# ESandML/SSL4GIE

Measured on AMD Instinct MI355X. Metric: images/sec/GPU (fwd+bwd) ViT-B 224² bs=256 at 1/2/4/8 MI355X; % MFMA peak, higher is better.
Workload: dtype bf16; 1 GPU; ViT-B MAE pretrain (mae_vit_base_patch16, norm_pix_loss, mask 0.75) fwd+bwd+grad-allreduce+AdamW, 224x224 synthetic N(0,1) images resident in HBM; batch_per_gpu=256, global_batch=256, parallelism=dp1, optimizer=AdamW(0.9,0.95) wd 0.05 (ssl4gie_amd.optim.ArenaAdamW)

## Files before the change

include/ssl4gie_hip.h:

```cpp
#ifndef SSL4GIE_HIP_H
#define SSL4GIE_HIP_H
#include <stddef.h>
#include <stdint.h>
#ifdef __cplusplus
extern "C" {
#endif

#define SSL4GIE_F32 0
#define SSL4GIE_BF16 1
#define SSL4GIE_EARG 1000
#define SSL4GIE_EPEER 1001

int ssl4gie_abi_version(void);

int ssl4gie_layernorm_fwd(const float* x, const float* gamma, const float* beta, void* y,
                          int y_dtype, float* mean, float* rstd, int rows, int cols, float eps,
                          void* stream);
size_t ssl4gie_layernorm_bwd_workspace_bytes(int rows, int cols);
int ssl4gie_layernorm_bwd(const void* dy, int dy_dtype, const float* x, const float* gamma,
                          const float* mean, const float* rstd, const float* dres, float* dx,
                          void* dx_lp, int lp_dtype, float* dgamma, float* dbeta, int accumulate,
                          float* workspace, int rows, int cols, void* stream);

size_t ssl4gie_colsum_workspace_bytes(int rows, int cols);
int ssl4gie_colsum(const void* x, int dtype, float* out, int accumulate, float* workspace,
                   int rows, int cols, long long ld, void* stream);

enum {
    SSL4GIE_EPI_NONE = 0,
    SSL4GIE_EPI_BIAS = 1,
    SSL4GIE_EPI_BIAS_GELU = 2,
    SSL4GIE_EPI_BIAS_RESIDUAL = 3,
    SSL4GIE_EPI_DGELU = 4,
    SSL4GIE_EPI_BIAS_GELU_GRAD = 5,
    SSL4GIE_EPI_MUL_AUX = 6,
    SSL4GIE_EPI_RELU_MASK_AUX = 7,
    SSL4GIE_EPI_ADD_AUX = 8,
    SSL4GIE_EPI_AFFINE_AUX_RELU = 9
};
typedef struct ssl4gie_conv3x3_geom {
    int B, H, W, C;
    int stride;
    int relu;
} ssl4gie_conv3x3_geom;

typedef struct ssl4gie_gemm_desc {
    int M, N, K;
    int batch1, batch2;
    const void* A;
    long long sAm, sAk, sAb1, sAb2;
    const void* B;
    long long sBk, sBn, sBb1, sBb2;
    void* C;
    long long ldc, sCb1, sCb2;
    int dtype_ab;
    int dtype_c;
    float alpha;
    int epilogue;
    const float* bias;
    const float* residual;
    long long ldr;
    const void* aux;
    void* out2;
    int accumulate;
    float* colsum_a;
    const ssl4gie_conv3x3_geom* conv;
    float* colstats;
    const float* scale;
    int relu;
} ssl4gie_gemm_desc;
size_t ssl4gie_gemm_workspace_bytes(const ssl4gie_gemm_desc* d);
int ssl4gie_gemm(const ssl4gie_gemm_desc* d, void* workspace, size_t workspace_bytes,
                 void* stream);
size_t ssl4gie_gemm_tn_pair_workspace_bytes(const ssl4gie_gemm_desc* a, const ssl4gie_gemm_desc* b);
int ssl4gie_gemm_tn_pair(const ssl4gie_gemm_desc* a, const ssl4gie_gemm_desc* b, void* workspace,
                         size_t workspace_bytes, void* stream);
size_t ssl4gie_gemm_tn_group_workspace_bytes(const ssl4gie_gemm_desc* descs, int n);
int ssl4gie_gemm_tn_group(const ssl4gie_gemm_desc* descs, int n, void* workspace,
                          size_t workspace_bytes, void* stream);

size_t ssl4gie_attn_workspace_bytes(int dtype, int B, int N, int H, int hd);
int ssl4gie_attn_fwd(const void* qkv, void* out, float* lse, int dtype, int B, int N, int H,
                     int hd, void* workspace, void* stream);
int ssl4gie_attn_bwd(const void* qkv, const void* out, const void* dout, const float* lse,
                     void* dqkv, int dtype, int B, int N, int H, int hd, void* workspace,
                     void* stream);

int ssl4gie_cast(const float* src, void* dst, int dst_dtype, long long n, void* stream);
int ssl4gie_cast_transpose(const float* src, void* dst, int dst_dtype, int rows, int cols,
                           void* stream);
int ssl4gie_cast_transpose_batch(const float* src, void* dst, const long long* mat_off,
                                 const int* mat_rows, const int* mat_cols, const int* tile_start,
                                 int S, int total_tiles, void* stream);
int ssl4gie_add_cast(const float* a, const float* b, float* out, void* out_lp, int lp_dtype,
                     long long n, void* stream);

int ssl4gie_mask_argsort(const float* noise, long long* ids_shuffle, long long* ids_restore,
                         float* mask, int B, int L, int len_keep, void* stream);
int ssl4gie_patch_gather(const float* img, const long long* ids, void* out, int out_dtype,
                         int B, int C, int H, int W, int p, int nsel, long long ids_stride,
                         int order, void* stream);
int ssl4gie_tokens_assemble(const void* y, int y_dtype, const float* cls, const float* pos,
                            const long long* ids, long long ids_stride, float* x, int B,
                            int nsel, int D, void* stream);
int ssl4gie_tokens_assemble_bwd(const float* dx, void* dy, int dy_dtype, float* dcls,
                                int accumulate, int B, int nsel, int D, void* stream);
int ssl4gie_decoder_assemble(const void* y, int y_dtype, const float* mask_token,
                             const float* dpos, const long long* ids_restore, float* xd, int B,
                             int L, int nkeep, int D, void* stream);
size_t ssl4gie_decoder_assemble_bwd_workspace_bytes(int B, int L, int D);
int ssl4gie_decoder_assemble_bwd(const float* dxd, const long long* ids_shuffle, void* dy,
                                 int dy_dtype, float* dmask_token, int accumulate,
                                 float* workspace, int B, int L, int nkeep, int D, void* stream);
int ssl4gie_mae_loss(const float* pred, const float* img, const float* mask, float* per_patch,
                     float* dpred, const float* gpp, float gscale_host, int norm_pix,
                     int has_cls, int B, int C, int H, int W, int p, void* stream);

typedef struct ssl4gie_block_weights {
    const float *ln1_g, *ln1_b, *ln2_g, *ln2_b;
    const float *bqkv, *bproj, *bfc1, *bfc2;
    const void *wqkv, *wproj, *wfc1, *wfc2;
    const void *wqkv_t, *wproj_t, *wfc1_t, *wfc2_t;
} ssl4gie_block_weights;
typedef struct ssl4gie_block_grads {
    float *ln1_g, *ln1_b, *ln2_g, *ln2_b;
    float *bqkv, *bproj, *bfc1, *bfc2;
    float *wqkv, *wproj, *wfc1, *wfc2;
} ssl4gie_block_grads;
typedef struct ssl4gie_block_act {
    float *mean1, *rstd1, *mean2, *rstd2;
    void* h1;
    void* qkv;
    void* attn;
    float* lse;
    float* xmid;
    void* h2;
    void* u;
    void* g;
} ssl4gie_block_act;
typedef struct ssl4gie_block_dims {
    int B, N, D, H, F;
    int dtype;
    float eps;
} ssl4gie_block_dims;
size_t ssl4gie_block_workspace_bytes(const ssl4gie_block_dims* d);
int ssl4gie_block_fwd(const ssl4gie_block_dims* d, const ssl4gie_block_weights* w,
                      const ssl4gie_block_act* a, const float* x_in, float* x_out,
                      void* workspace, void* stream);
#define SSL4GIE_BWD_ACCUMULATE 1
#define SSL4GIE_BWD_DEFER_WGRAD 2
#define SSL4GIE_BWD_NO_JOIN 4
#define SSL4GIE_BWD_SLOT(s) (((s) & 3) << 4)
int ssl4gie_block_bwd(const ssl4gie_block_dims* d, const ssl4gie_block_weights* w,
                      const ssl4gie_block_act* a, const ssl4gie_block_grads* g,
                      const float* x_in, const float* dx_out, const void* dx_out_lp,
                      float* dx_in, void* dx_in_lp, int accumulate, void* workspace,
                      void* stream);
int ssl4gie_set_wgrad_stream(int on);
int ssl4gie_block_wgrad_descs(const ssl4gie_block_dims* d, const ssl4gie_block_act* a,
                              const ssl4gie_block_grads* g, const void* dy, void* workspace,
                              int accumulate, ssl4gie_gemm_desc* out4);
int ssl4gie_wgrad_group(const ssl4gie_gemm_desc* descs, int n, void* workspace, size_t workspace_bytes,
                        int slot, void* stream);
int ssl4gie_wgrad_wait(int slot, void* stream);
int ssl4gie_set_compute_cus(int n);

int ssl4gie_conv3x3_weight_pack(const float* w, void* out, int dtype, int Cout, int Cin, int mode, int ld,
                                void* stream);
int ssl4gie_conv3x3_weight_pack_batch(const void* const* w, void* const* out, const int* Cout, const int* Cin,
                                      const int* mode, const int* ld, int n, int dtype, void* stream);
int ssl4gie_conv3x3_wgrad_unpack(const float* dw2, float* dw, int Cout, int Cin, int ld, int accumulate,
                                 void* stream);
int ssl4gie_im2col3x3(const void* x, void* cols, int dtype, int B, int H, int W, int C, int stride,
                      int relu, long long ld, void* stream);
int ssl4gie_col2im3x3(const void* dcols, void* dx, int dtype, int B, int H, int W, int C,
                      int stride, long long ld, void* stream);
int ssl4gie_conv3x3_direct_ok(int B, int H, int W, int Cin, int Cout);
int ssl4gie_conv3x3_direct_tiles(int B, int H, int W);
int ssl4gie_conv3x3_direct_fwd(const void* x, const void* w2, const float* bias,
                               const void* relu_mask, void* y, float* colstats, int B, int H, int W,
                               int Cin, int Cout, int relu_in, void* stream);
int ssl4gie_conv3x3_direct_wgrad_ok(int B, int H, int W, int Cin, int Cout);
size_t ssl4gie_conv3x3_direct_wgrad_workspace_bytes(int B, int H, int W, int Cin, int Cout);
int ssl4gie_conv3x3_direct_wgrad(const void* dy, const void* x, float* dw2, float* dbias,
                                 void* workspace, size_t workspace_bytes, int B, int H, int W, int Cin,
                                 int Cout, int relu_in, int accumulate, void* stream);
int ssl4gie_conv3x3_direct_fwd_affine(const void* x, const float* in_coef, const void* w2, const float* bias,
                                      void* y, float* colstats, int B, int H, int W, int Cin, int Cout,
                                      int relu_in, void* stream);
int ssl4gie_conv3x3_direct_wgrad_affine(const void* dy, const void* x, const float* in_coef, float* dw2,
                                        float* dbias, void* workspace, size_t workspace_bytes, int B, int H,
                                        int W, int Cin, int Cout, int relu_in, int accumulate, void* stream);
size_t ssl4gie_stem7x7_packed_bytes(int B, int H, int W);
int ssl4gie_stem7x7_pack(const float* img, void* packed, int B, int H, int W, void* stream);
int ssl4gie_stem7x7_tiles(int B, int H, int W);
int ssl4gie_stem7x7_fwd(const void* packed, const void* w2s, void* y, float* colstats, int B, int H,
                        int W, void* stream);
size_t ssl4gie_stem7x7_wgrad_workspace_bytes(int B, int H, int W);
int ssl4gie_stem7x7_wgrad(const void* dy, const void* packed, float* dw2s, void* workspace,
                          size_t workspace_bytes, int B, int H, int W, int accumulate, void* stream);
int ssl4gie_bilinear2x_fwd(const void* x, void* y, int dtype, int B, int H, int W, int C,
                           void* stream);
int ssl4gie_bilinear2x_bwd(const void* dy, void* dx, int dtype, int B, int H, int W, int C,
                           void* stream);
int ssl4gie_pixel_shuffle(const void* g, const float* bias, void* y, int dtype, int B, int H, int W,
                          int k, int C, void* stream);
int ssl4gie_pixel_unshuffle(const void* dy, void* dg, int dtype, int B, int H, int W, int k, int C,
                            void* stream);
int ssl4gie_tokens_to_map(const float* z, void* x, int dtype, int B, int L, int D, void* stream);
int ssl4gie_map_to_tokens(const void* dx, float* dz, int dtype, int B, int L, int D, void* stream);
int ssl4gie_eltwise(int op, const void* a, const void* b, const void* c, void* out, int dtype,
                    long long n, void* stream);
int ssl4gie_depth_head_fwd(const void* x, const float* w, const float* bias, float* y, int dtype,
                           long long M, int C, void* stream);
size_t ssl4gie_depth_head_bwd_workspace_bytes(long long M, int C);
int ssl4gie_depth_head_bwd(const void* x, const float* w, const float* y, const float* dy, void* dx,
                           float* dw, float* db, int accumulate, float* workspace, int dtype,
                           long long M, int C, void* stream);

int ssl4gie_stem_im2col7x7(const float* img, void* cols, int dtype, int B, int H, int W,
                           long long ld, void* stream);
int ssl4gie_subsample2(const void* x, void* y, int dtype, int B, int H, int W, int C, int backward,
                       void* stream);
size_t ssl4gie_bn_workspace_bytes(long long rows, int C);
int ssl4gie_bn_fwd(const void* x, const float* gamma, const float* beta, const void* res, void* y,
                   float* mean, float* rstd, float* running_mean, float* running_var,
                   float momentum, float eps, int relu, int training, float* workspace, int dtype,
                   long long rows, int C, void* stream);
int ssl4gie_bn_bwd(const void* dy, const void* y, const void* x, const float* gamma,
                   const float* mean, const float* rstd, void* dx, void* dres, float* dgamma,
                   float* dbeta, int accumulate, int relu, float* workspace, int dtype,
                   long long rows, int C, void* stream);
int ssl4gie_bn_bwd_xmask(const void* dy, const void* x, const float* gamma, const float* beta,
                         const float* mean, const float* rstd, void* dx, float* dgamma, float* dbeta,
                         int accumulate, float* workspace, int dtype, long long rows, int C, void* stream);
int ssl4gie_bn_fwd_partials_bits(const void* x, const float* partial, int parts, const float* gamma,
                                 const float* beta, const void* res, void* y, unsigned char* relu_bits,
                                 float* mean, float* rstd, float* running_mean, float* running_var,
                                 float momentum, float eps, float* workspace, int dtype, long long rows, int C,
                                 void* stream);
int ssl4gie_bn_bwd_bits(const void* dy, const unsigned char* relu_bits, const void* x, const float* gamma,
                        const float* mean, const float* rstd, void* dx, void* dres, float* dgamma, float* dbeta,
                        int accumulate, float* workspace, int dtype, long long rows, int C, void* stream);
int ssl4gie_bn_stats(const void* x, float* mean, float* var, float* workspace, int dtype,
                     long long rows, int C, void* stream);
int ssl4gie_bn_combine_stats(const float* gathered, int world, int C, float eps, float momentum,
                             float* running_mean, float* running_var, float* mean, float* rstd, float* total,
                             void* stream);
int ssl4gie_bn_bwd_reduce(const void* dy, const void* y, const void* x, const float* mean,
                          const float* rstd, void* dres, float* sums, int relu, float* workspace,
                          int dtype, long long rows, int C, void* stream);
int ssl4gie_bn_bwd_apply(const void* dy, const void* y, const void* x, const float* gamma,
                         const float* mean, const float* rstd, const float* sums, float inv_count,
                         void* dx, int relu, float* workspace, int dtype, long long rows, int C,
                         void* stream);
int ssl4gie_bn_bwd_reduce_xmask(const void* dy, const void* x, const float* gamma, const float* beta,
                                const float* mean, const float* rstd, float* sums, float* workspace, int dtype,
                                long long rows, int C, void* stream);
int ssl4gie_bn_bwd_apply_xmask(const void* dy, const void* x, const float* gamma, const float* beta,
                               const float* mean, const float* rstd, const float* sums, float inv_count, void* dx,
                               float* workspace, int dtype, long long rows, int C, void* stream);
int ssl4gie_bn_coef_stats(const float* mean, const float* rstd, const float* gamma, const float* beta, float* coef,
                          int C, void* stream);
int ssl4gie_bn_apply_bits(const void* x, const float* coef, const void* res, void* y, unsigned char* relu_bits,
                          int dtype, long long rows, int C, void* stream);
int ssl4gie_bn_bwd_reduce_bits(const void* dy, const unsigned char* relu_bits, const void* x, const float* mean,
                               const float* rstd, void* dres, float* sums, float* workspace, int dtype,
                               long long rows, int C, void* stream);
int ssl4gie_ema_update(float* dst, const float* src, float m, long long n, void* stream);
int ssl4gie_bn_fwd_partials(const void* x, const float* partial, int parts, const float* gamma,
                            const float* beta, const void* res, void* y, float* mean, float* rstd,
                            float* running_mean, float* running_var, float momentum, float eps,
                            int relu, float* workspace, int dtype, long long rows, int C,
                            void* stream);
int ssl4gie_bn_coef_partials(const float* partial, int parts, const float* gamma, const float* beta,
                             float* mean, float* rstd, float* running_mean, float* running_var,
                             float momentum, float eps, float* coef, float* workspace, long long rows, int C,
                             void* stream);
int ssl4gie_bn_stats_partials(const float* partial, int parts, float* mean, float* var,
                              float* workspace, long long rows, int C, void* stream);
int ssl4gie_maxpool3x3s2_fwd(const void* x, void* y, unsigned char* arg, int dtype, int B, int H,
                             int W, int C, void* stream);
int ssl4gie_maxpool3x3s2_bwd(const void* dy, const unsigned char* arg, void* dx, int dtype, int B,
                             int H, int W, int C, void* stream);
int ssl4gie_bn_maxpool3x3s2_fwd(const void* x, const float* coef, int relu, void* y, unsigned char* arg,
                                int dtype, int B, int H, int W, int C, void* stream);
int ssl4gie_avgpool_fwd(const void* x, float* y, int dtype, int B, int HW, int C, void* stream);
int ssl4gie_avgpool_bwd(const float* dy, void* dx, int dtype, int B, int HW, int C, void* stream);

int ssl4gie_adamw_arena(float* p, const float* g, float* m, float* v, const long long* seg_start,
                        const float* seg_lr, const float* seg_wd, int S, float beta1, float beta2,
                        float eps, int step, long long n, void* stream);
int ssl4gie_adamw_arena_lp(float* p, const float* g, float* m, float* v, const long long* seg_start,
                           const float* seg_lr, const float* seg_wd, int S, float beta1, float beta2,
                           float eps, int step, long long n, void* lp_bf16, void* stream);
int ssl4gie_adamw_arena_range(float* p, const float* g, float* m, float* v, const long long* seg_start,
                              const float* seg_lr, const float* seg_wd, int S, float beta1, float beta2,
                              float eps, int step, long long lo, long long hi, void* lp_bf16,
                              void* stream);
size_t ssl4gie_lars_workspace_bytes(int S);
int ssl4gie_lars_arena(float* p, const float* g, float* mu, const long long* seg_start,
                       const float* seg_lr, const float* seg_wd, const float* seg_mat, int S,
                       float momentum, float trust, float* workspace, long long n, void* stream);

int ssl4gie_normalize_u8(const unsigned char* img, float* out, const float* mean, const float* std,
                         int B, int H, int W, void* stream);

int ssl4gie_maxpool2x2_fwd(const void* x, void* y, int dtype, int B, int H, int W, int C,
                           void* stream);
int ssl4gie_maxpool2x2_bwd(const void* x, const void* dy, void* dx, int dtype, int B, int H, int W,
                           int C, void* stream);
int ssl4gie_gelu_map(const void* x, const void* dy, void* out, int dtype, long long n, void* stream);
size_t ssl4gie_map_layernorm_workspace_bytes(int B);
int ssl4gie_map_layernorm_fwd(const void* x, const float* w, const float* bias, void* y, float* mean,
                              float* rstd, float eps, float* workspace, int dtype, int B, long long M,
                              void* stream);
int ssl4gie_map_layernorm_bwd(const void* x, const void* dy, const float* w, const float* mean,
                              const float* rstd, void* dx, float* dw, float* db, int accumulate,
                              float* workspace, int dtype, int B, long long M, void* stream);

#define SSL4GIE_PROF_KINDS 7
int ssl4gie_prof_begin(int max_launches);
int ssl4gie_prof_collect(double* ms, double* flops, long long* launches);
int ssl4gie_prof_end(void);

size_t ssl4gie_ssi_loss_workspace_bytes(int B, int H, int W);
int ssl4gie_ssi_loss(const float* pred, const float* target, float* loss, float* dpred, int B, int H,
                     int W, float alpha, int scales, void* workspace, void* stream);
size_t ssl4gie_dice_loss_workspace_bytes(int B);
int ssl4gie_dice_loss(const float* logits, const float* target, float* loss, float* dlogits, int B,
                      long long n, float smooth, void* workspace, void* stream);

int ssl4gie_debug_nt256_stamps(void* dst, size_t bytes);

typedef struct ssl4gie_ar_handle ssl4gie_ar_handle;
size_t ssl4gie_allreduce_direct_blob_bytes(void);
int ssl4gie_allreduce_direct_init(int rank, int world, size_t max_elems, void* export_blob,
                                  ssl4gie_ar_handle** out);
int ssl4gie_allreduce_direct_connect(ssl4gie_ar_handle* h, const void* all_blobs);
int ssl4gie_allreduce_direct_enqueue(ssl4gie_ar_handle* h, float* grad, size_t n_elems, float scale,
                                     void* stream);
int ssl4gie_allgather_direct_enqueue(ssl4gie_ar_handle* h, const float* src, size_t n_elems, float* dst,
                                     void* stream);
unsigned ssl4gie_allreduce_direct_error(const ssl4gie_ar_handle* h);
int ssl4gie_allreduce_direct_set_timeout(ssl4gie_ar_handle* h, double seconds);
int ssl4gie_allreduce_direct_destroy(ssl4gie_ar_handle* h);

#ifdef __cplusplus
}
#endif
#endif
```

ssl4gie_amd/_lib.py:

```python
from __future__ import annotations

import ctypes as C
import os

_HERE = os.path.dirname(os.path.abspath(__file__))
LIB_PATH = os.path.join(_HERE, "libssl4gie_hip.so")
_dbg = os.environ.get("SSL4GIE_DEBUG_LIB", "")
if _dbg == "1" or _dbg.startswith("x"):
    LIB_PATH = os.path.join(_HERE, "libssl4gie_hip_dbg.so" if _dbg == "1" else f"libssl4gie_hip_{_dbg}.so")
    import sys as _sys
    print(f"ssl4gie_amd: SSL4GIE_DEBUG_LIB=1 -> loading the DEBUG library {LIB_PATH}", file=_sys.stderr)

ABI_VERSION = 7

PROF_KINDS = 7

F32, BF16 = 0, 1
BWD_ACCUMULATE, BWD_DEFER_WGRAD, BWD_NO_JOIN = 1, 2, 4
EPI_NONE, EPI_BIAS, EPI_BIAS_GELU, EPI_BIAS_RESIDUAL, EPI_DGELU, EPI_BIAS_GELU_GRAD, EPI_MUL_AUX, \
    EPI_RELU_MASK_AUX, EPI_ADD_AUX, EPI_AFFINE_AUX_RELU = range(10)

vp, i32, i64, f32, sz = C.c_void_p, C.c_int, C.c_longlong, C.c_float, C.c_size_t


class Conv3x3Geom(C.Structure):
    _fields_ = [("B", i32), ("H", i32), ("W", i32), ("C", i32), ("stride", i32), ("relu", i32)]


class GemmDesc(C.Structure):
    _fields_ = [
        ("M", i32), ("N", i32), ("K", i32), ("batch1", i32), ("batch2", i32),
        ("A", vp), ("sAm", i64), ("sAk", i64), ("sAb1", i64), ("sAb2", i64),
        ("B", vp), ("sBk", i64), ("sBn", i64), ("sBb1", i64), ("sBb2", i64),
        ("C", vp), ("ldc", i64), ("sCb1", i64), ("sCb2", i64),
        ("dtype_ab", i32), ("dtype_c", i32), ("alpha", f32), ("epilogue", i32),
        ("bias", vp), ("residual", vp), ("ldr", i64), ("aux", vp), ("out2", vp),
        ("accumulate", i32), ("colsum_a", vp), ("conv", C.POINTER(Conv3x3Geom)),
        ("colstats", vp), ("scale", vp), ("relu", i32),
    ]


_W_F32 = ("ln1_g", "ln1_b", "ln2_g", "ln2_b", "bqkv", "bproj", "bfc1", "bfc2")
_W_LP = ("wqkv", "wproj", "wfc1", "wfc2", "wqkv_t", "wproj_t", "wfc1_t", "wfc2_t")
_G_ALL = _W_F32 + ("wqkv", "wproj", "wfc1", "wfc2")
_ACT = ("mean1", "rstd1", "mean2", "rstd2", "h1", "qkv", "attn", "lse", "xmid", "h2", "u", "g")


class BlockWeights(C.Structure):
    _fields_ = [(n, vp) for n in _W_F32 + _W_LP]


class BlockGrads(C.Structure):
    _fields_ = [(n, vp) for n in _G_ALL]


class BlockAct(C.Structure):
    _fields_ = [(n, vp) for n in _ACT]


class BlockDims(C.Structure):
    _fields_ = [("B", i32), ("N", i32), ("D", i32), ("H", i32), ("F", i32), ("dtype", i32),
                ("eps", f32)]


PROTOTYPES = {
    "ssl4gie_abi_version": (i32, []),
    "ssl4gie_layernorm_fwd": (i32, [vp, vp, vp, vp, i32, vp, vp, i32, i32, f32, vp]),
    "ssl4gie_layernorm_bwd_workspace_bytes": (sz, [i32, i32]),
    "ssl4gie_layernorm_bwd": (i32, [vp, i32, vp, vp, vp, vp, vp, vp, vp, i32, vp, vp, i32, vp,
                                    i32, i32, vp]),
    "ssl4gie_colsum_workspace_bytes": (sz, [i32, i32]),
    "ssl4gie_colsum": (i32, [vp, i32, vp, i32, vp, i32, i32, i64, vp]),
    "ssl4gie_gemm_workspace_bytes": (sz, [C.POINTER(GemmDesc)]),
    "ssl4gie_gemm": (i32, [C.POINTER(GemmDesc), vp, sz, vp]),
    "ssl4gie_attn_workspace_bytes": (sz, [i32, i32, i32, i32, i32]),
    "ssl4gie_attn_fwd": (i32, [vp, vp, vp, i32, i32, i32, i32, i32, vp, vp]),
    "ssl4gie_attn_bwd": (i32, [vp, vp, vp, vp, vp, i32, i32, i32, i32, i32, vp, vp]),
    "ssl4gie_cast": (i32, [vp, vp, i32, i64, vp]),
    "ssl4gie_cast_transpose": (i32, [vp, vp, i32, i32, i32, vp]),
    "ssl4gie_cast_transpose_batch": (i32, [vp, vp, vp, vp, vp, vp, i32, i32, vp]),
    "ssl4gie_add_cast": (i32, [vp, vp, vp, vp, i32, i64, vp]),
    "ssl4gie_mask_argsort": (i32, [vp, vp, vp, vp, i32, i32, i32, vp]),
    "ssl4gie_patch_gather": (i32, [vp, vp, vp, i32, i32, i32, i32, i32, i32, i32, i64, i32, vp]),
    "ssl4gie_tokens_assemble": (i32, [vp, i32, vp, vp, vp, i64, vp, i32, i32, i32, vp]),
    "ssl4gie_tokens_assemble_bwd": (i32, [vp, vp, i32, vp, i32, i32, i32, i32, vp]),
    "ssl4gie_decoder_assemble": (i32, [vp, i32, vp, vp, vp, vp, i32, i32, i32, i32, vp]),
    "ssl4gie_decoder_assemble_bwd_workspace_bytes": (sz, [i32, i32, i32]),
    "ssl4gie_decoder_assemble_bwd": (i32, [vp, vp, vp, i32, vp, i32, vp, i32, i32, i32, i32, vp]),
    "ssl4gie_mae_loss": (i32, [vp, vp, vp, vp, vp, vp, f32, i32, i32, i32, i32, i32, i32, i32, vp]),
    "ssl4gie_im2col3x3": (i32, [vp, vp, i32, i32, i32, i32, i32, i32, i32, i64, vp]),
    "ssl4gie_col2im3x3": (i32, [vp, vp, i32, i32, i32, i32, i32, i32, i64, vp]),
    "ssl4gie_conv3x3_direct_ok": (i32, [i32, i32, i32, i32, i32]),
    "ssl4gie_conv3x3_direct_tiles": (i32, [i32, i32, i32]),
    "ssl4gie_conv3x3_direct_fwd": (i32, [vp, vp, vp, vp, vp, vp, i32, i32, i32, i32, i32, i32, vp]),
    "ssl4gie_conv3x3_direct_wgrad_ok": (i32, [i32, i32, i32, i32, i32]),
    "ssl4gie_conv3x3_direct_wgrad_workspace_bytes": (sz, [i32, i32, i32, i32, i32]),
    "ssl4gie_conv3x3_direct_wgrad": (i32, [vp, vp, vp, vp, vp, sz, i32, i32, i32, i32, i32, i32, i32, vp]),
    "ssl4gie_conv3x3_direct_wgrad_affine": (i32, [vp, vp, vp, vp, vp, vp, sz, i32, i32, i32, i32, i32, i32, i32, vp]),
    "ssl4gie_conv3x3_direct_fwd_affine": (i32, [vp, vp, vp, vp, vp, vp, i32, i32, i32, i32, i32, i32, vp]),
    "ssl4gie_stem7x7_packed_bytes": (sz, [i32, i32, i32]),
    "ssl4gie_stem7x7_pack": (i32, [vp, vp, i32, i32, i32, vp]),
    "ssl4gie_stem7x7_tiles": (i32, [i32, i32, i32]),
    "ssl4gie_stem7x7_fwd": (i32, [vp, vp, vp, vp, i32, i32, i32, vp]),
    "ssl4gie_stem7x7_wgrad_workspace_bytes": (sz, [i32, i32, i32]),
    "ssl4gie_stem7x7_wgrad": (i32, [vp, vp, vp, vp, sz, i32, i32, i32, i32, vp]),
    "ssl4gie_bilinear2x_fwd": (i32, [vp, vp, i32, i32, i32, i32, i32, vp]),
    "ssl4gie_bilinear2x_bwd": (i32, [vp, vp, i32, i32, i32, i32, i32, vp]),
    "ssl4gie_pixel_shuffle": (i32, [vp, vp, vp, i32, i32, i32, i32, i32, i32, vp]),
    "ssl4gie_pixel_unshuffle": (i32, [vp, vp, i32, i32, i32, i32, i32, i32, vp]),
    "ssl4gie_tokens_to_map": (i32, [vp, vp, i32, i32, i32, i32, vp]),
    "ssl4gie_map_to_tokens": (i32, [vp, vp, i32, i32, i32, i32, vp]),
    "ssl4gie_eltwise": (i32, [i32, vp, vp, vp, vp, i32, i64, vp]),
    "ssl4gie_depth_head_fwd": (i32, [vp, vp, vp, vp, i32, i64, i32, vp]),
    "ssl4gie_depth_head_bwd_workspace_bytes": (sz, [i64, i32]),
    "ssl4gie_depth_head_bwd": (i32, [vp, vp, vp, vp, vp, vp, vp, i32, vp, i32, i64, i32, vp]),
    "ssl4gie_stem_im2col7x7": (i32, [vp, vp, i32, i32, i32, i32, i64, vp]),
    "ssl4gie_subsample2": (i32, [vp, vp, i32, i32, i32, i32, i32, i32, vp]),
    "ssl4gie_bn_workspace_bytes": (sz, [i64, i32]),
    "ssl4gie_bn_fwd": (i32, [vp, vp, vp, vp, vp, vp, vp, vp, vp, f32, f32, i32, i32, vp, i32, i64, i32, vp]),
    "ssl4gie_bn_bwd": (i32, [vp, vp, vp, vp, vp, vp, vp, vp, vp, vp, i32, i32, vp, i32, i64, i32, vp]),
    "ssl4gie_bn_stats": (i32, [vp, vp, vp, vp, i32, i64, i32, vp]),
    "ssl4gie_bn_fwd_partials_bits": (i32, [vp, vp, i32, vp, vp, vp, vp, vp, vp, vp, vp, vp, f32, f32, vp, i32, i64,
                                           i32, vp]),
    "ssl4gie_bn_bwd_bits": (i32, [vp, vp, vp, vp, vp, vp, vp, vp, vp, vp, i32, vp, i32, i64, i32, vp]),
    "ssl4gie_bn_bwd_xmask": (i32, [vp, vp, vp, vp, vp, vp, vp, vp, vp, i32, vp, i32, i64, i32, vp]),
    "ssl4gie_bn_bwd_reduce_xmask": (i32, [vp, vp, vp, vp, vp, vp, vp, vp, i32, i64, i32, vp]),
    "ssl4gie_bn_bwd_apply_xmask": (i32, [vp, vp, vp, vp, vp, vp, vp, f32, vp, vp, i32, i64, i32, vp]),
    "ssl4gie_bn_bwd_reduce": (i32, [vp, vp, vp, vp, vp, vp, vp, i32, vp, i32, i64, i32, vp]),
    "ssl4gie_bn_coef_stats": (i32, [vp, vp, vp, vp, vp, i32, vp]),
    "ssl4gie_bn_apply_bits": (i32, [vp, vp, vp, vp, vp, i32, i64, i32, vp]),
    "ssl4gie_bn_bwd_reduce_bits": (i32, [vp, vp, vp, vp, vp, vp, vp, vp, i32, i64, i32, vp]),
    "ssl4gie_bn_bwd_apply": (i32, [vp, vp, vp, vp, vp, vp, vp, f32, vp, i32, vp, i32, i64, i32, vp]),
    "ssl4gie_ema_update": (i32, [vp, vp, f32, i64, vp]),
    "ssl4gie_maxpool3x3s2_fwd": (i32, [vp, vp, vp, i32, i32, i32, i32, i32, vp]),
    "ssl4gie_bn_maxpool3x3s2_fwd": (i32, [vp, vp, i32, vp, vp, i32, i32, i32, i32, i32, vp]),
    "ssl4gie_maxpool3x3s2_bwd": (i32, [vp, vp, vp, i32, i32, i32, i32, i32, vp]),
    "ssl4gie_avgpool_fwd": (i32, [vp, vp, i32, i32, i32, i32, vp]),
    "ssl4gie_avgpool_bwd": (i32, [vp, vp, i32, i32, i32, i32, vp]),
    "ssl4gie_bn_coef_partials": (i32, [vp, i32, vp, vp, vp, vp, vp, vp, f32, f32, vp, vp, i64, i32, vp]),
    "ssl4gie_bn_fwd_partials": (i32, [vp, vp, i32, vp, vp, vp, vp, vp, vp, vp, vp, f32, f32, i32, vp, i32, i64,
                                      i32, vp]),
    "ssl4gie_bn_stats_partials": (i32, [vp, i32, vp, vp, vp, i64, i32, vp]),
    "ssl4gie_adamw_arena": (i32, [vp, vp, vp, vp, vp, vp, vp, i32, f32, f32, f32, i32, i64, vp]),
    "ssl4gie_adamw_arena_lp": (i32, [vp, vp, vp, vp, vp, vp, vp, i32, f32, f32, f32, i32, i64, vp, vp]),
    "ssl4gie_adamw_arena_range": (i32, [vp, vp, vp, vp, vp, vp, vp, i32, f32, f32, f32, i32, i64, i64, vp, vp]),
    "ssl4gie_lars_workspace_bytes": (sz, [i32]),
    "ssl4gie_lars_arena": (i32, [vp, vp, vp, vp, vp, vp, vp, i32, f32, f32, vp, i64, vp]),
    "ssl4gie_normalize_u8": (i32, [vp, vp, C.POINTER(C.c_float), C.POINTER(C.c_float), i32, i32, i32, vp]),
    "ssl4gie_maxpool2x2_fwd": (i32, [vp, vp, i32, i32, i32, i32, i32, vp]),
    "ssl4gie_maxpool2x2_bwd": (i32, [vp, vp, vp, i32, i32, i32, i32, i32, vp]),
    "ssl4gie_gelu_map": (i32, [vp, vp, vp, i32, i64, vp]),
    "ssl4gie_map_layernorm_workspace_bytes": (sz, [i32]),
    "ssl4gie_map_layernorm_fwd": (i32, [vp, vp, vp, vp, vp, vp, f32, vp, i32, i32, i64, vp]),
    "ssl4gie_map_layernorm_bwd": (i32, [vp, vp, vp, vp, vp, vp, vp, vp, i32, vp, i32, i32, i64, vp]),
    "ssl4gie_gemm_tn_pair_workspace_bytes": (sz, [vp, vp]),
    "ssl4gie_gemm_tn_pair": (i32, [vp, vp, vp, sz, vp]),
    "ssl4gie_gemm_tn_group_workspace_bytes": (sz, [vp, i32]),
    "ssl4gie_gemm_tn_group": (i32, [vp, i32, vp, sz, vp]),
    "ssl4gie_block_wgrad_descs": (i32, [C.POINTER(BlockDims), C.POINTER(BlockAct), C.POINTER(BlockGrads), vp, vp,
                                        i32, vp]),
    "ssl4gie_wgrad_group": (i32, [vp, i32, vp, sz, i32, vp]),
    "ssl4gie_wgrad_wait": (i32, [i32, vp]),
    "ssl4gie_set_wgrad_stream": (i32, [i32]),
    "ssl4gie_set_compute_cus": (i32, [i32]),
    "ssl4gie_ssi_loss_workspace_bytes": (sz, [i32, i32, i32]),
    "ssl4gie_ssi_loss": (i32, [vp, vp, vp, vp, i32, i32, i32, f32, i32, vp, vp]),
    "ssl4gie_dice_loss_workspace_bytes": (sz, [i32]),
    "ssl4gie_dice_loss": (i32, [vp, vp, vp, vp, i32, i64, f32, vp, vp]),
    "ssl4gie_allreduce_direct_blob_bytes": (sz, []),
    "ssl4gie_allreduce_direct_init": (i32, [i32, i32, sz, vp, C.POINTER(vp)]),
    "ssl4gie_allreduce_direct_connect": (i32, [vp, vp]),
    "ssl4gie_allreduce_direct_enqueue": (i32, [vp, vp, sz, f32, vp]),
    "ssl4gie_allgather_direct_enqueue": (i32, [vp, vp, sz, vp, vp]),
    "ssl4gie_bn_combine_stats": (i32, [vp, i32, i32, f32, f32, vp, vp, vp, vp, vp, vp]),
    "ssl4gie_allreduce_direct_error": (C.c_uint, [vp]),
    "ssl4gie_allreduce_direct_set_timeout": (i32, [vp, C.c_double]),
    "ssl4gie_allreduce_direct_destroy": (i32, [vp]),
    "ssl4gie_conv3x3_weight_pack_batch": (i32, [vp, vp, vp, vp, vp, vp, i32, i32, vp]),
    "ssl4gie_conv3x3_weight_pack": (i32, [vp, vp, i32, i32, i32, i32, i32, vp]),
    "ssl4gie_conv3x3_wgrad_unpack": (i32, [vp, vp, i32, i32, i32, i32, vp]),
    "ssl4gie_debug_nt256_stamps": (i32, [vp, sz]),
    "ssl4gie_prof_begin": (i32, [i32]),
    "ssl4gie_prof_collect": (i32, [vp, vp, vp]),
    "ssl4gie_prof_end": (i32, []),
    "ssl4gie_block_workspace_bytes": (sz, [C.POINTER(BlockDims)]),
    "ssl4gie_block_fwd": (i32, [C.POINTER(BlockDims), C.POINTER(BlockWeights),
                                C.POINTER(BlockAct), vp, vp, vp, vp]),
    "ssl4gie_block_bwd": (i32, [C.POINTER(BlockDims), C.POINTER(BlockWeights),
                                C.POINTER(BlockAct), C.POINTER(BlockGrads), vp, vp, vp, vp, vp,
                                i32, vp, vp]),
}

_lib = None


class HipExtensionMissing(RuntimeError):
    pass


def load():
    global _lib
    if _lib is not None:
        return _lib
    if not os.path.exists(LIB_PATH):
        raise HipExtensionMissing(
            f"{LIB_PATH} not found: build it with `make -C ssl4gie_amd/csrc` "
            "(or `python -c 'import __graft_entry__ as g; g.build()'`). "
            "ssl4gie_amd has no CPU / eager fallback.")
    lib = C.CDLL(LIB_PATH)
    for name, (res, args) in PROTOTYPES.items():
        fn = getattr(lib, name)
        fn.restype = res
        fn.argtypes = args
    got = lib.ssl4gie_abi_version()
    if got != ABI_VERSION:
        raise HipExtensionMissing(
            f"{LIB_PATH} has ABI revision {got}, this package binds revision {ABI_VERSION}: "
            "rebuild it (`make -C ssl4gie_amd/csrc`)")
    _lib = lib
    return lib


def check(rc: int, what: str):
    if rc != 0:
        kind = {1000: "invalid argument",
                1001: "a peer of the direct all-reduce did not arrive in time (sticky)"}.get(rc, f"hipError_t {rc}")
        raise RuntimeError(f"libssl4gie_hip: {what} failed ({kind})")
```

ssl4gie_amd/csrc/gemm256.h:

```cpp
#pragma once
#include "gemm_internal.h"

#define P_BM 256
#define P_BN 256
#define P_BK 64
#define P_HALF 16384
#define P_BUF 65536
#define P_STG_WAVE 4096
#define P_LDS_BYTES (2 * P_BUF + 8 * P_STG_WAVE)

DEVI int p_swz(int r) { return (r >> 1) & 7; }

DEVI unsigned p_lds_addr(const void* p) {
    return (unsigned)(uintptr_t)(__attribute__((address_space(3))) const char*)p;
}

DEVI void p_glds2(const void* sbase, unsigned v0, unsigned v1, unsigned l0, unsigned l1) {
    unsigned keep;
    asm volatile(
        "s_mov_b32 %0, m0\n\t"
        "s_mov_b32 m0, %4\n\t"
        "s_nop 0\n\t"
        "global_load_lds_dwordx4 %2, %1\n\t"
        "s_mov_b32 m0, %5\n\t"
        "s_nop 0\n\t"
        "global_load_lds_dwordx4 %3, %1\n\t"
        "s_mov_b32 m0, %0"
        : "=&s"(keep)
        : "s"(sbase), "v"(v0), "v"(v1), "s"(l0), "s"(l1)
        : "memory");
}

DEVI void p_glds1(const void* sbase, unsigned v0, unsigned l0) {
    unsigned keep;
    asm volatile(
        "s_mov_b32 %0, m0\n\t"
        "s_mov_b32 m0, %3\n\t"
        "s_nop 0\n\t"
        "global_load_lds_dwordx4 %2, %1\n\t"
        "s_mov_b32 m0, %0"
        : "=&s"(keep)
        : "s"(sbase), "v"(v0), "s"(l0)
        : "memory");
}

DEVI void p_glds1_dword(const void* sbase, unsigned v0, unsigned l0) {
    unsigned keep;
    asm volatile(
        "s_mov_b32 %0, m0\n\t"
        "s_mov_b32 m0, %3\n\t"
        "s_nop 0\n\t"
        "global_load_lds_dword %2, %1\n\t"
        "s_mov_b32 m0, %0"
        : "=&s"(keep)
        : "s"(sbase), "v"(v0), "s"(l0)
        : "memory");
}

DEVI void p_glds2v(const void* a0, const void* a1, unsigned l0, unsigned l1) {
    unsigned keep;
    asm volatile(
        "s_mov_b32 %0, m0\n\t"
        "s_mov_b32 m0, %3\n\t"
        "s_nop 0\n\t"
        "global_load_lds_dwordx4 %1, off\n\t"
        "s_mov_b32 m0, %4\n\t"
        "s_nop 0\n\t"
        "global_load_lds_dwordx4 %2, off\n\t"
        "s_mov_b32 m0, %0"
        : "=&s"(keep)
        : "v"(a0), "v"(a1), "s"(l0), "s"(l1)
        : "memory");
}

DEVI unsigned p_fastdiv(unsigned n, unsigned mg, unsigned sh) { return __umulhi(n, mg) >> sh; }

DEVI bf16x8 p_relu8(bf16x8 v) {
    typedef __attribute__((ext_vector_type(8))) short s16x8_t;
    const s16x8_t z = {0, 0, 0, 0, 0, 0, 0, 0};
    return __builtin_bit_cast(bf16x8, __builtin_elementwise_max(__builtin_bit_cast(s16x8_t, v), z));
}

#ifndef P_EPI_XPOSE_SWAP
#define P_EPI_XPOSE_SWAP true
#endif
#ifndef P_EPI_PRIO_MODE
#define P_EPI_PRIO_MODE 0
#endif
#define P_MFMA(a, b, c) __builtin_amdgcn_mfma_f32_16x16x32_bf16((a), (b), (c), 0, 0, 0)

template <bool NT, class V> DEVI void est(V* p, V v) {
    if constexpr (NT) __builtin_nontemporal_store(v, p);
    else *p = v;
}
template <bool NT> DEVI void est4(float* p, f32x4 v) { est<NT>((f32x4*)p, v); }
template <bool NT> DEVI void est4(bf16_t* p, f32x4 v) {
    u32x2 r;
    r[0] = pack_bf2(v[0], v[1]);
    r[1] = pack_bf2(v[2], v[3]);
    est<NT>((u32x2*)p, r);
}

template <bool FULL, bool RESID, int NJ = 4, bool NT = false>
DEVI void p_store_f32(f32x4 (&acc)[8][4], char* stg, const float alpha, const f32x4 bias_t ,
                      const float* __restrict__ residual, const long long ldr, const bool accumulate,
                      float* __restrict__ C, const long long ldc, int rbase, int cbase, int M, int N,
                      int lane) {
    const int r16 = lane & 15, g4 = lane >> 4;
    const int R0 = lane >> 4, Cc = lane & 15;
    const int gn = cbase + 4 * Cc;
    const bool mine = NJ == 4 || Cc < 4 * NJ;
    constexpr int PF = NJ == 3 ? 3 : 2;
    f32x4 rs[PF][4];
    auto fetch = [&](int mt, f32x4 (&dst)[4]) {
#pragma unroll
        for (int q = 0; q < 4; ++q) {
            const int gm = rbase + 16 * mt + R0 + 4 * q;
            dst[q] = (mine && (FULL || (gm < M && gn < N))) ? ld4(residual + (size_t)gm * ldr + gn)
                                                            : f32x4{0, 0, 0, 0};
        }
    };
    if constexpr (RESID) {
#pragma unroll
        for (int mt = 0; mt < PF; ++mt) fetch(mt, rs[mt]);
    }
    auto put = [&](int mt) {
#pragma unroll
        for (int nt = 0; nt < NJ; ++nt) {
            const f32x4 v = acc[mt][nt] * alpha;
            const int c = nt * 4 + g4;
            *(f32x4*)(stg + r16 * 256 + ((c ^ r16) << 4)) = v;
        }
    };
    put(0);
#pragma unroll
    for (int mt = 0; mt < 8; ++mt) {
        f32x4 w[4];
#pragma unroll
        for (int q = 0; q < 4; ++q) {
            const int R = R0 + 4 * q;
            w[q] = *(const f32x4*)(stg + R * 256 + ((Cc ^ R) << 4));
        }
        __builtin_amdgcn_sched_barrier(0);
        if (mt + 1 < 8) put(mt + 1);
        __builtin_amdgcn_sched_barrier(0);
#pragma unroll
        for (int q = 0; q < 4; ++q) {
            const int R = R0 + 4 * q;
            const int gm = rbase + 16 * mt + R;
            w[q] += bias_t;
            if constexpr (RESID) w[q] += rs[mt % PF][q];
            if (mine && (FULL || (gm < M && gn < N))) {
                float* c = C + (size_t)gm * ldc + gn;
                if (accumulate) w[q] += ld4(c);
                est4<NT>(c, w[q]);
            }
        }
        if constexpr (RESID) {
            if (mt + PF < 8) fetch(mt + PF, rs[mt % PF]);
        }
    }
}

template <bool FULL, int AUXF, int NJ = 4, bool NT = false>
DEVI void p_store_bf16_aux(f32x4 (&acc)[8][4], char* stg, const float alpha,
                           const bf16_t* __restrict__ aux, bf16_t* __restrict__ C,
                           const long long ldc, int rbase, int cbase, int M, int N, int lane,
                           const float* __restrict__ scale = nullptr, const float* __restrict__ shift = nullptr,
                           const int relu = 0) {
    const int r16 = lane & 15, g4 = lane >> 4;
    const int R0 = lane >> 4, Cc = lane & 15;
    const int gn = cbase + 4 * Cc;
    const bool mine = NJ == 4 || Cc < 4 * NJ;
    [[maybe_unused]] f32x4 sc4 = {1, 1, 1, 1}, sh4 = {0, 0, 0, 0};
    [[maybe_unused]] const bool has_aux = AUXF != 5 || aux != nullptr;
    if constexpr (AUXF == 5) {
        if (mine && (FULL || gn < N)) { sc4 = ld4(scale + gn); sh4 = ld4(shift + gn); }
    }
    constexpr int PF = AUXF == 5 ? 2 : 4;
    u32x2 ax[PF][4];
    auto fetch = [&](int mt, u32x2 (&dst)[4]) {
#pragma unroll
        for (int q = 0; q < 4; ++q) {
            const int gm = rbase + 16 * mt + R0 + 4 * q;
            dst[q] = (has_aux && mine && (FULL || (gm < M && gn < N))) ? *(const u32x2*)(aux + (size_t)gm * ldc + gn)
                                                                       : u32x2{0, 0};
        }
    };
#pragma unroll
    for (int mt = 0; mt < PF; ++mt) fetch(mt, ax[mt]);
    auto put = [&](int mt) {
#pragma unroll
        for (int nt = 0; nt < NJ; ++nt) {
            const f32x4 v = acc[mt][nt] * alpha;
            const int c = nt * 4 + g4;
            *(f32x4*)(stg + r16 * 256 + ((c ^ r16) << 4)) = v;
        }
    };
    put(0);
#pragma unroll
    for (int mt = 0; mt < 8; ++mt) {
        f32x4 w[4];
#pragma unroll
        for (int q = 0; q < 4; ++q) {
            const int R = R0 + 4 * q;
            w[q] = *(const f32x4*)(stg + R * 256 + ((Cc ^ R) << 4));
        }
        __builtin_amdgcn_sched_barrier(0);
        if (mt + 1 < 8) put(mt + 1);
        __builtin_amdgcn_sched_barrier(0);
#pragma unroll
        for (int q = 0; q < 4; ++q) {
            const int R = R0 + 4 * q;
            const int gm = rbase + 16 * mt + R;
            const u32x2 r = ax[mt % PF][q];
            f32x4 u = {__uint_as_float(r[0] << 16), __uint_as_float(r[0] & 0xffff0000u),
                       __uint_as_float(r[1] << 16), __uint_as_float(r[1] & 0xffff0000u)};
            if constexpr (AUXF == 2) {
#pragma unroll
                for (int j = 0; j < 4; ++j) u[j] = dgelu_fast(u[j]);
            }
            if constexpr (AUXF == 3) {
#pragma unroll
                for (int j = 0; j < 4; ++j) w[q][j] = u[j] > 0.f ? w[q][j] : 0.f;
            } else if constexpr (AUXF == 4) {
                w[q] += u;
            } else if constexpr (AUXF == 5) {
                w[q] = w[q] * sc4 + sh4 + u;
                if (relu) {
#pragma unroll
                    for (int j = 0; j < 4; ++j) w[q][j] = w[q][j] > 0.f ? w[q][j] : 0.f;
                }
            } else {
                w[q] *= u;
            }
            if (mine && (FULL || (gm < M && gn < N))) est4<NT>(C + (size_t)gm * ldc + gn, w[q]);
        }
        if (mt + PF < 8) fetch(mt + PF, ax[mt % PF]);
    }
}

DEVI float p_fold_lanes8(float v) {
    const unsigned b0 = __float_as_uint(v);
    v += __uint_as_float((unsigned)__builtin_amdgcn_update_dpp(0, (int)b0, 0x128 , 0xf, 0xf, false));
    const unsigned b1 = __float_as_uint(v);
    const u32x2 s1 = __builtin_amdgcn_permlane16_swap(b1, b1, false, false);
    v = __uint_as_float(s1[0]) + __uint_as_float(s1[1]);
    const unsigned b2 = __float_as_uint(v);
    const u32x2 s2 = __builtin_amdgcn_permlane32_swap(b2, b2, false, false);
    return __uint_as_float(s2[0]) + __uint_as_float(s2[1]);
}

#define P_TAB_BYTES 16384
struct GeluTabQ { f32x4 u; unsigned e[4]; };
DEVI void p_gelu_tab_read(const f32x4 u, const char* tab, GeluTabQ& q) {
    typedef unsigned short u16x2_t __attribute__((ext_vector_type(2)));
    q.u = u;
#pragma unroll
    for (int h = 0; h < 2; ++h) {
        const unsigned p = pack_bf2(u[2 * h], u[2 * h + 1]);
        const u16x2_t m = __builtin_bit_cast(u16x2_t, p & 0x7fff7fffu);
        u16x2_t t = __builtin_elementwise_sub_sat(m, (u16x2_t)(unsigned short)0x3980);
        t = __builtin_elementwise_min(t, (u16x2_t)(unsigned short)2047);
        const unsigned T = (((p >> 4) & 0x08000800u) | __builtin_bit_cast(unsigned, t)) << 2;
        q.e[2 * h] = *(const unsigned*)(tab + (T & 0xffffu));
        q.e[2 * h + 1] = *(const unsigned*)(tab + (T >> 16));
    }
}
DEVI float p_mix_lo16(float x, unsigned e) {
    float r;
    asm("v_fma_mix_f32 %0, %1, %2, 0 op_sel_hi:[0,1,0]" : "=v"(r) : "v"(x), "v"(e));
    return r;
}
DEVI void p_gelu_tab_finish(const GeluTabQ& q, unsigned (&d)[2], unsigned (&g)[2]) {
#pragma unroll
    for (int h = 0; h < 2; ++h) {
        g[h] = pack_bf2(p_mix_lo16(q.u[2 * h], q.e[2 * h]), p_mix_lo16(q.u[2 * h + 1], q.e[2 * h + 1]));
        d[h] = __builtin_amdgcn_perm(q.e[2 * h + 1], q.e[2 * h], 0x07060302u);
    }
}

template <typename TC, int MODE, bool FULL, bool STATS, bool BIAS_LDS = false, int NJ = 4, bool NT = false, bool TAB = false>
DEVI void p_epilogue(f32x4 (&acc)[8][4], char* stg, const float alpha,
                     const float* __restrict__ bias, const float* __restrict__ residual,
                     const long long ldr, const bf16_t* __restrict__ aux, bf16_t* __restrict__ out2,
                     const int accumulate, TC* __restrict__ C, long long ldc, int rbase, int cbase,
                     int M, int N, int lane, float* __restrict__ colstats,
                     unsigned long long* tstamp = nullptr ,
                     const int prio_mode = P_EPI_PRIO_MODE ,
                     const bool xpose_swap = P_EPI_XPOSE_SWAP ,
                     const char* tab = nullptr ) {
    const int r16 = lane & 15, g4 = lane >> 4;
    constexpr bool HAS_BIAS = MODE == SSL4GIE_EPI_BIAS || MODE == SSL4GIE_EPI_BIAS_GELU ||
                              MODE == SSL4GIE_EPI_BIAS_RESIDUAL || MODE == SSL4GIE_EPI_BIAS_GELU_GRAD;
    f32x4 bias4[4], bias_t = {0, 0, 0, 0};
#pragma unroll
    for (int nt = 0; nt < 4; ++nt) bias4[nt] = f32x4{0, 0, 0, 0};
    if constexpr (HAS_BIAS && sizeof(TC) == 2) {
#pragma unroll
        for (int nt = 0; nt < NJ; ++nt) {
            const int n = cbase + 16 * nt + 4 * g4;
            if constexpr (BIAS_LDS) {
                const f32x4 t = *(const f32x4*)(stg + (16 * nt + 4 * g4) * 4);
                bias4[nt] = bias ? t : f32x4{0, 0, 0, 0};
            } else {
                if (bias && (FULL || n < N)) bias4[nt] = ld4(bias + n);
            }
        }
    }
    if constexpr (HAS_BIAS && sizeof(TC) == 4) {
        const int c4 = 4 * (lane & 15);
        if constexpr (BIAS_LDS) {
            const f32x4 t = *(const f32x4*)(stg + c4 * 4);
            bias_t = bias ? t : f32x4{0, 0, 0, 0};
        } else {
            if (bias && (FULL || cbase + c4 < N)) bias_t = ld4(bias + cbase + c4);
        }
    }
    if constexpr (BIAS_LDS) __builtin_amdgcn_sched_barrier(0);
    if constexpr (sizeof(TC) == 2 && MODE == SSL4GIE_EPI_AFFINE_AUX_RELU) {
        p_store_bf16_aux<FULL, 5, NJ, NT>(acc, stg, alpha, aux, (bf16_t*)C, ldc, rbase, cbase, M, N, lane,
                                      residual , bias , accumulate );
    } else if constexpr (sizeof(TC) == 2 && (MODE == SSL4GIE_EPI_DGELU || MODE == SSL4GIE_EPI_MUL_AUX ||
                                      MODE == SSL4GIE_EPI_RELU_MASK_AUX || MODE == SSL4GIE_EPI_ADD_AUX)) {
        constexpr int AUXF = MODE == SSL4GIE_EPI_DGELU ? 2
                           : (MODE == SSL4GIE_EPI_RELU_MASK_AUX ? 3 : (MODE == SSL4GIE_EPI_ADD_AUX ? 4 : 1));
        p_store_bf16_aux<FULL, AUXF, NJ, NT>(acc, stg, alpha, aux, (bf16_t*)C, ldc, rbase, cbase, M, N, lane);
    } else if constexpr (sizeof(TC) == 2) {
        const int R0 = lane >> 3, Cc = lane & 7;
        auto put = [&](int base, int nt, const f32x4& x) {
            u32x2 pk;
            pk[0] = pack_bf2(x[0], x[1]);
            pk[1] = pack_bf2(x[2], x[3]);
            const int c = nt * 2 + (g4 >> 1);
            *(u32x2*)(stg + base + r16 * 128 + ((c ^ (r16 & 7)) << 4) + ((g4 & 1) << 3)) = pk;
        };
        f32x2 cs[4], cq[4];
        if constexpr (STATS) {
#pragma unroll
            for (int j = 0; j < 4; ++j) cs[j] = cq[j] = f32x2{0.f, 0.f};
        }
        constexpr bool PAIR = MODE == SSL4GIE_EPI_BIAS_GELU_GRAD || MODE == SSL4GIE_EPI_BIAS_GELU;
        const bool mine = NJ == 4 || Cc < 2 * NJ;
        auto stage = [&](int mt) {
#pragma unroll
            for (int nt = 0; nt < NJ; ++nt) {
                const f32x4 v = acc[mt][nt] * alpha + bias4[nt];
                if constexpr (MODE == SSL4GIE_EPI_BIAS_GELU_GRAD) {
                    f32x4 g, d;
                    gelu_grad4_fast(v, d, g);
                    put(0, nt, d);
                    put(2048, nt, g);
                } else if constexpr (MODE == SSL4GIE_EPI_BIAS_GELU) {
                    f32x4 g;
#pragma unroll
                    for (int q = 0; q < 4; ++q) g[q] = gelu_fast(v[q]);
                    put(0, nt, v);
                    put(2048, nt, g);
                } else {
                    put(0, nt, v);
                }
            }
        };
        auto fetch = [&](int base, u32x4 (&w)[2]) {
#pragma unroll
            for (int hh = 0; hh < 2; ++hh) {
                const int R = R0 + 8 * hh;
                w[hh] = *(const u32x4*)(stg + base + R * 128 + ((Cc ^ (R & 7)) << 4));
            }
        };
        auto store = [&](const u32x4 (&w)[2], bf16_t* __restrict__ dst, int mt, bool stats) {
#pragma unroll
            for (int hh = 0; hh < 2; ++hh) {
                const int R = R0 + 8 * hh;
                const int gm = rbase + 16 * mt + R, gn = cbase + 8 * Cc;
                if (mine && (FULL || (gm < M && gn < N))) {
                    if (!STATS || dst) est<NT>((u32x4*)(dst + (size_t)gm * ldc + gn), w[hh]);
                    if constexpr (STATS) {
                        if (stats && !(prio_mode & 8)) {
#pragma unroll
                            for (int j = 0; j < 4; ++j) {
                                const f32x2 v = {__uint_as_float(w[hh][j] << 16), __uint_as_float(w[hh][j] & 0xffff0000u)};
                                cs[j] += v;
                                cq[j] = v * v + cq[j];
                            }
                        }
                    }
                }
            }
        };
        if constexpr (PAIR && NJ == 4 && TAB) {
            static_assert(!STATS, "the table form exists for the GELU pair only");
            GeluTabQ qa[2], qb[2];
            auto rd = [&](int i, GeluTabQ& a, GeluTabQ& b) {
                const int mt = i >> 1, np = i & 1;
                p_gelu_tab_read(acc[mt][2 * np] * alpha + bias4[2 * np], tab, a);
                p_gelu_tab_read(acc[mt][2 * np + 1] * alpha + bias4[2 * np + 1], tab, b);
            };
            rd(0, qa[0], qb[0]);
#pragma unroll
            for (int i = 0; i < 16; ++i) {
                const int mt = i >> 1, np = i & 1;
                if (i + 1 < 16) rd(i + 1, qa[(i + 1) & 1], qb[(i + 1) & 1]);
                unsigned dA[2], gA[2], dB[2], gB[2];
                p_gelu_tab_finish(qa[i & 1], dA, gA);
                p_gelu_tab_finish(qb[i & 1], dB, gB);
                auto xq = [&](const unsigned (&a)[2], const unsigned (&b)[2]) -> u32x4 {
                    const u32x2 s1 = __builtin_amdgcn_permlane16_swap(a[0], b[0], false, false);
                    const u32x2 s2 = __builtin_amdgcn_permlane16_swap(a[1], b[1], false, false);
                    return u32x4{s1[0], s2[0], s1[1], s2[1]};
                };
                const u32x4 wg = xq(gA, gB);
                const int gm = rbase + 16 * mt + r16;
                const int gn = cbase + 32 * np + 16 * (g4 & 1) + 8 * (g4 >> 1);
                if constexpr (MODE == SSL4GIE_EPI_BIAS_GELU_GRAD) {
                    const u32x4 wd = xq(dA, dB);
                    if (FULL || (gm < M && gn < N)) {
                        est<NT>((u32x4*)((bf16_t*)C + (size_t)gm * ldc + gn), wd);
                        est<NT>((u32x4*)(out2 + (size_t)gm * ldc + gn), wg);
                    }
                } else {
                    const f32x4& uA = qa[i & 1].u;
                    const f32x4& uB = qb[i & 1].u;
                    const unsigned ua[2] = {pack_bf2(uA[0], uA[1]), pack_bf2(uA[2], uA[3])};
                    const unsigned ub[2] = {pack_bf2(uB[0], uB[1]), pack_bf2(uB[2], uB[3])};
                    const u32x4 wu = xq(ua, ub);
                    if (FULL || (gm < M && gn < N)) {
                        est<NT>((u32x4*)((bf16_t*)C + (size_t)gm * ldc + gn), wu);
                        est<NT>((u32x4*)(out2 + (size_t)gm * ldc + gn), wg);
                    }
                }
            }
            return;
        }
        if constexpr (PAIR && NJ == 4 && !TAB) {
            if (xpose_swap) {
#pragma unroll
                for (int mt = 0; mt < 8; ++mt) {
                    const int gm = rbase + 16 * mt + r16;
#pragma unroll
                    for (int np = 0; np < 2; ++np) {
                        f32x4 dA, gA, dB, gB;
                        const f32x4 vA = acc[mt][2 * np] * alpha + bias4[2 * np];
                        const f32x4 vB = acc[mt][2 * np + 1] * alpha + bias4[2 * np + 1];
                        if constexpr (MODE == SSL4GIE_EPI_BIAS_GELU_GRAD) {
                            gelu_grad4_fast(vA, dA, gA);
                            gelu_grad4_fast(vB, dB, gB);
                        } else {
                            dA = vA; dB = vB;
#pragma unroll
                            for (int q = 0; q < 4; ++q) { gA[q] = gelu_fast(vA[q]); gB[q] = gelu_fast(vB[q]); }
                        }
                        auto xp = [&](const f32x4& a, const f32x4& b) -> u32x4 {
                            const u32x2 s1 = __builtin_amdgcn_permlane16_swap(pack_bf2(a[0], a[1]), pack_bf2(b[0], b[1]), false, false);
                            const u32x2 s2 = __builtin_amdgcn_permlane16_swap(pack_bf2(a[2], a[3]), pack_bf2(b[2], b[3]), false, false);
                            return u32x4{s1[0], s2[0], s1[1], s2[1]};
                        };
                        const u32x4 wd = xp(dA, dB), wg = xp(gA, gB);
                        const int gn = cbase + 32 * np + 16 * (g4 & 1) + 8 * (g4 >> 1);
                        if (FULL || (gm < M && gn < N)) {
                            est<NT>((u32x4*)((bf16_t*)C + (size_t)gm * ldc + gn), wd);
                            est<NT>((u32x4*)(out2 + (size_t)gm * ldc + gn), wg);
                        }
                    }
                    if (tstamp) tstamp[mt] = __builtin_amdgcn_s_memrealtime();
                }
                return;
            }
        }
        const int wrow = (rbase >> 7) & 1;
        auto prio = [&](int blk) {
            if constexpr (PAIR) {
                const int pm = prio_mode & 3;
                const bool hi = pm == 1 ? wrow == 1
                              : pm == 2 ? ((blk & 1) == 0) == (wrow == 1)
                              : pm == 3 ? ((blk & 1) == 0) == (wrow == 0) : false;
                if (hi) __builtin_amdgcn_s_setprio(1);
                else __builtin_amdgcn_s_setprio(0);
            }
        };
        prio(0);
        stage(0);
#pragma unroll
        for (int mt = 0; mt < 8; ++mt) {
            u32x4 w0[2], w1[2];
            fetch(0, w0);
            if constexpr (PAIR) fetch(2048, w1);
            __builtin_amdgcn_sched_barrier(0);
            prio(mt + 1);
            if (mt + 1 < 8) stage(mt + 1);
            __builtin_amdgcn_sched_barrier(0);
            store(w0, (bf16_t*)C, mt, true);
            if constexpr (PAIR) store(w1, out2, mt, false);
            if (tstamp) tstamp[mt] = __builtin_amdgcn_s_memrealtime();
        }
        if constexpr (PAIR) __builtin_amdgcn_s_setprio(0);
        if constexpr (STATS) {
            if (!(prio_mode & 16))
            {
#pragma unroll
                for (int j = 0; j < 4; ++j) {
                    cs[j] = f32x2{p_fold_lanes8(cs[j][0]), p_fold_lanes8(cs[j][1])};
                    cq[j] = f32x2{p_fold_lanes8(cq[j][0]), p_fold_lanes8(cq[j][1])};
                }
            }
            const int gn = cbase + 8 * Cc;
            if (lane < 8 && mine && !(prio_mode & 32) && (FULL || (gn < N && rbase < M))) {
                float* p = colstats + (size_t)(rbase >> 7) * 2 * N + gn;
                st4(p, f32x4{cs[0][0], cs[0][1], cs[1][0], cs[1][1]});
                st4(p + 4, f32x4{cs[2][0], cs[2][1], cs[3][0], cs[3][1]});
                st4(p + N, f32x4{cq[0][0], cq[0][1], cq[1][0], cq[1][1]});
                st4(p + N + 4, f32x4{cq[2][0], cq[2][1], cq[3][0], cq[3][1]});
            }
        }
    } else {
        p_store_f32<FULL, MODE == SSL4GIE_EPI_BIAS_RESIDUAL, NJ, NT>(
            acc, stg, alpha, bias_t, residual, ldr, MODE == SSL4GIE_EPI_NONE && accumulate, (float*)C,
            ldc, rbase, cbase, M, N, lane);
    }
}
```

ssl4gie_amd/csrc/gemm_nt256.hip:

```cpp
#include "gemm256.h"
#include "gelu_table.h"
#include "prof.h"

#include <stdio.h>
#include <stdlib.h>
#include <type_traits>

#define NT256_DEFAULT_ROLE 0
#define NT256_DEFAULT_PH2 true

#define NT256_STAMP_WGS 16
#define NT256_STAMP_TILES 16
#ifdef SSL4GIE_DEBUG_KNOBS
__device__ unsigned long long g_nt256_stamps[NT256_STAMP_WGS][NT256_STAMP_TILES][16];

extern "C" int ssl4gie_debug_nt256_stamps(void* dst, size_t bytes) {
    REQUIRE(dst && bytes <= sizeof(g_nt256_stamps));
    HIP_RET(hipMemcpyFromSymbol(dst, HIP_SYMBOL(g_nt256_stamps), bytes));
    return 0;
}
#else
extern "C" int ssl4gie_debug_nt256_stamps(void*, size_t) { return ARG_ERR; }
#endif

template <typename TC, int MODE, int CONV, bool STATS = false, int ROLE = 0, int NJ = 4, bool PH2 = false,
          bool NTS = false , bool TAB = false>
__global__ __launch_bounds__(512, 2) void gemm_bf16_nt256_kernel(
    const bf16_t* __restrict__ A, long long lda, const bf16_t* __restrict__ B, long long ldb,
    TC* __restrict__ C, long long ldc, int M, int N, int K, int tiles_n, int ntiles, EpiArgs e,
    int dbg_arg ,
    ConvK cg) {
#ifdef SSL4GIE_DEBUG_KNOBS
    const int dbg = dbg_arg & 15;
    const int dbg_prio = dbg_arg >> 4;
#else
    constexpr int dbg = 0;
#endif
    extern __shared__ __attribute__((aligned(16))) char smem[];
    const int t = threadIdx.x, lane = t & 63;
    const int wave = __builtin_amdgcn_readfirstlane(t >> 6);
    const int wr = wave >> 2, wc = wave & 3;
    const int G = gridDim.x;
    const int pos = xcd_remap(blockIdx.x, G);
    const int my_tiles = (ntiles - pos + G - 1) / G;
    auto tile_of = [&](int ti) { return pos + ti * G; };
    const int nk = K / P_BK;
    const int total_kt = my_tiles * nk;
    const float e_alpha = e.alpha;
    const float* e_bias = e.bias;
    const float* e_residual = e.residual;
    const long long e_ldr = e.ldr;
    const bf16_t* e_aux = (const bf16_t*)e.aux;
    bf16_t* e_out2 = (bf16_t*)e.out2;
    const int e_accumulate = e.accumulate;
    float* e_colstats = e.colstats;

    constexpr int NP = ROLE ? 4 : 2;
    const int pbase = ROLE ? wc * 4 : wave * 2;
    const bool loader = ROLE == 0 || wr == 1;
    unsigned vo[4][2], co[2];
    unsigned yo[2][2];
    static_assert(CONV == 0 || ROLE == 0, "the gathered operand keeps the two-piece ownership");
    static_assert(NJ == 4 || ((NJ == 3 || NJ == 2) && ROLE == 0 && CONV == 0), "256 x 192 / 256 x 128: plain operands, ROLE 0");
    static_assert(!TAB || (NJ == 4 && ROLE == 0 && CONV == 0 && !STATS && sizeof(TC) == 2 &&
                           (MODE == SSL4GIE_EPI_BIAS_GELU || MODE == SSL4GIE_EPI_BIAS_GELU_GRAD)),
                  "the table form exists for the GELU pair on the 256 x 256 tile");
    constexpr int WN = 16 * NJ;
    constexpr int BN = 4 * WN;
#pragma unroll
    for (int J = 0; J < 4; ++J) vo[J][0] = vo[J][1] = 0;
    yo[0][0] = yo[0][1] = yo[1][0] = yo[1][1] = 0;
#pragma unroll
    for (int i = 0; i < 2; ++i) {
        const int lr = (pbase + i) * 8 + (lane >> 3);
        co[i] = (unsigned)(((lane & 7) ^ p_swz(lr)) * 16);
    }
    const unsigned a_step = (unsigned)(16 * lda * 2), b_step = (unsigned)(16 * ldb * 2);
    const unsigned a_last = (unsigned)((long long)(M - 1) * lda * 2), b_last = (unsigned)((long long)(N - 1) * ldb * 2);
    const int c_H = cg.H, c_W = cg.W, c_C = cg.C, c_Wo = cg.Wo, c_HoWo = cg.HoWo, c_s = cg.stride;
    const unsigned c_mgw = cg.mg_wo, c_shw = cg.sh_wo, c_mgh = cg.mg_hw, c_shh = cg.sh_hw;
    const char* c_zero = (const char*)cg.zero;
    const int c_cpt = c_C / P_BK;
    auto point_at = [&](int ti) {
        const int tile = tile_of(ti);
        const int sm0 = (tile / tiles_n) * P_BM, sn0 = (tile % tiles_n) * BN;
        auto offs = [&](int i, int h, bool is_a) -> unsigned {
            if (NJ == 3 && !is_a && h == 1) {
                const int lr1 = wave * 8 + (lane >> 3);
                int rb = sn0 + (lr1 >> 4) * WN + 32 + (lr1 & 15);
                rb = rb < N ? rb : N - 1;
                return (unsigned)((long long)rb * ldb * 2) + (unsigned)(((lane & 7) ^ p_swz(lr1)) * 16);
            }
            const int lr = (pbase + i) * 8 + (lane >> 3);
            if (is_a) {
                int ra = sm0 + (lr >> 6) * 128 + h * 64 + (lr & 63);
                ra = ra < M ? ra : M - 1;
                if constexpr (CONV != 0) return (unsigned)ra;
                return (unsigned)((long long)ra * lda * 2) + (ROLE == 0 ? co[i] : 0u);
            }
            int rb = sn0 + (lr >> 5) * WN + h * 32 + (lr & 31);
            rb = rb < N ? rb : N - 1;
            return (unsigned)((long long)rb * ldb * 2) + (ROLE == 0 ? co[i] : 0u);
        };
#pragma unroll
        for (int i = 0; i < 2; ++i) {
            vo[0][i] = offs(i, 0, false);
            vo[1][i] = offs(i, 0, true);
            vo[2][i] = offs(i, 1, false);
            vo[3][i] = offs(i, 1, true);
        }
        if constexpr (CONV != 0) {
            auto pix = [&](unsigned& v, unsigned& yx, int i) {
                const int lr = (pbase + i) * 8 + (lane >> 3);
                const int c = (lane & 7) ^ p_swz(lr);
                const unsigned m = v;
                const unsigned b = p_fastdiv(m, c_mgh, c_shh);
                const unsigned r = m - b * (unsigned)c_HoWo;
                const unsigned oy = p_fastdiv(r, c_mgw, c_shw);
                const unsigned ox = r - oy * (unsigned)c_Wo;
                const int y0 = (int)oy * c_s - 1, x0 = (int)ox * c_s - 1;
                v = (unsigned)(((((int)b * c_H + y0) * c_W + x0) * c_C + c * 8) * 2);
                yx = ((unsigned)y0 << 16) | ((unsigned)x0 & 0xffffu);
            };
#pragma unroll
            for (int i = 0; i < 2; ++i) {
                pix(vo[1][i], yo[0][i], i);
                pix(vo[3][i], yo[1][i], i);
            }
        }
    };
    const unsigned lds0 = __builtin_amdgcn_readfirstlane(p_lds_addr(smem) + pbase * 1024);
    int s_ktg = 0, s_kt = 0, s_ti = 0;
    int s_dy = 0, s_dx = 0, s_cib = 0;
    auto issue = [&](auto Jc) {
        constexpr int J = decltype(Jc)::value;
        if (!loader) return;
        if (s_ktg < total_kt && dbg != 7) {
            const unsigned dst = lds0 + (s_ktg & 1) * P_BUF + J * P_HALF;
            const bf16_t* base = ((J & 1) ? A : B) + (size_t)(dbg == 11 ? 0 : s_kt) * P_BK;
            if constexpr (CONV != 0 && (J & 1)) {
                const unsigned va = vo[J][0], vb = vo[J][1];
                const unsigned ya = yo[J >> 1][0], yb = yo[J >> 1][1];
                const int tapoff = ((s_dy * c_W + s_dx) * c_C + s_cib * P_BK) * 2;
                auto src = [&](unsigned o, unsigned yx) -> const char* {
                    const int y = ((int)yx >> 16) + s_dy, x = (int)(short)(yx & 0xffffu) + s_dx;
                    const bool ok = (unsigned)y < (unsigned)c_H && (unsigned)x < (unsigned)c_W;
                    return ok ? (const char*)A + (long long)((int)o + tapoff) : c_zero;
                };
                p_glds2v(src(va, ya), src(vb, yb), dst, dst + 1024);
            } else {
                if constexpr (NJ == 2 && J == 2) {
                } else if constexpr (NJ == 3 && J == 2) {
                    p_glds1(base, vo[J][0], dst - pbase * 1024 + wave * 1024);
                } else if constexpr (ROLE == 0) {
                    p_glds2(base, vo[J][0], vo[J][1], dst, dst + 1024);
                } else {
                    p_glds2(base, vo[J][0] + co[0], vo[J][1] + co[1], dst, dst + 1024);
                    const unsigned step = (J & 1) ? a_step : b_step, last = (J & 1) ? a_last : b_last;
                    const unsigned r2 = vo[J][0] + step, r3 = vo[J][1] + step;
                    p_glds2(base, (r2 < last ? r2 : last) + co[0], (r3 < last ? r3 : last) + co[1], dst + 2048,
                            dst + 3072);
                }
            }
        }
        if (J == 3) {
            ++s_ktg;
            if constexpr (CONV != 0) {
                if (++s_cib == c_cpt) {
                    s_cib = 0;
                    if (++s_dx == 3) { s_dx = 0; ++s_dy; }
                }
            }
            if (++s_kt == nk) {
                s_kt = 0;
                s_dy = 0; s_dx = 0; s_cib = 0;
                if (++s_ti < my_tiles) point_at(s_ti);
            }
        }
    };
    auto stream_wait = [&](bool more) {
        if (!loader) return;
        if (more) asm volatile("s_waitcnt vmcnt(%0)" ::"n"(NJ == 3 ? 5 : (NJ == 2 ? 4 : 3 * NP)) : "memory");
        else asm volatile("s_waitcnt vmcnt(0)" ::: "memory");
    };
    using I0 = std::integral_constant<int, 0>;
    using I1 = std::integral_constant<int, 1>;
    using I2 = std::integral_constant<int, 2>;
    using I3 = std::integral_constant<int, 3>;

    const int l15 = lane & 15, lg = lane >> 4;
    const int sw = p_swz(l15);
    const int offA = (wr * 64 + l15) * 128, offB = (wc * 32 + l15) * 128;
    const int offB1 = NJ == 3 ? (wc * 16 + l15) * 128 : offB;
    const int ch0 = ((0 * 4 + lg) ^ sw) << 4, ch1 = ((1 * 4 + lg) ^ sw) << 4;
    auto ldA = [&](int buf, int h, int mi, int ks) -> bf16x8 {
        return *(const bf16x8*)(smem + buf * P_BUF + (h ? 3 : 1) * P_HALF + offA + mi * 2048 +
                                (ks ? ch1 : ch0));
    };
    auto ldB = [&](int buf, int h, int ni, int ks) -> bf16x8 {
        return *(const bf16x8*)(smem + buf * P_BUF + (h ? 2 : 0) * P_HALF + (h ? offB1 : offB) + ni * 2048 +
                                (ks ? ch1 : ch0));
    };

    f32x4 acc[8][4];
#pragma unroll
    for (int i = 0; i < 8; ++i)
#pragma unroll
        for (int j = 0; j < NJ; ++j) acc[i][j] = f32x4{0, 0, 0, 0};
    bf16x8 a[4][2], b0[2][2], b1[2][2];
    constexpr int NI1 = NJ == 3 ? 1 : (NJ == 2 ? 0 : 2);

    auto mm = [&](auto QMc, auto QNc, auto MI0c, auto MI1c, bf16x8 (&bb)[2][2]) {
        constexpr int QM = decltype(QMc)::value, QN = decltype(QNc)::value;
        constexpr int MI0 = decltype(MI0c)::value, MI1 = decltype(MI1c)::value;
#pragma unroll
        for (int ks = 0; ks < 2; ++ks)
#pragma unroll
            for (int mi = MI0; mi < MI1; ++mi)
#pragma unroll
                for (int ni = 0; ni < (QN == 1 ? NI1 : 2); ++ni)
                    acc[QM * 4 + mi][QN * 2 + ni] =
                        P_MFMA(bb[ni][ks], a[mi][ks], acc[QM * 4 + mi][QN * 2 + ni]);
    };
    using I4 = std::integral_constant<int, 4>;
    auto mma = [&](auto PHc) {
        constexpr int PH = decltype(PHc)::value;
        if (dbg == 7) return;
        __builtin_amdgcn_s_setprio(1);
        if constexpr (CONV == 2 && (PH == 0 || PH == 2)) {
#pragma unroll
            for (int mi = 0; mi < 4; ++mi)
#pragma unroll
                for (int ks = 0; ks < 2; ++ks) a[mi][ks] = p_relu8(a[mi][ks]);
        }
        if constexpr (NJ == 2) {
            if constexpr (PH == 0) mm(I0{}, I0{}, I0{}, I4{}, b0);
            if constexpr (PH == 3) mm(I1{}, I0{}, I0{}, I4{}, b0);
        } else if constexpr (NJ == 4) {
            if constexpr (PH == 0) mm(I0{}, I0{}, I0{}, I4{}, b0);
            if constexpr (PH == 1) mm(I0{}, I1{}, I0{}, I4{}, b1);
            if constexpr (PH == 2) mm(I1{}, I1{}, I0{}, I4{}, b1);
            if constexpr (PH == 3) mm(I1{}, I0{}, I0{}, I4{}, b0);
        } else {
            if constexpr (PH == 0) mm(I0{}, I0{}, I0{}, I3{}, b0);
            if constexpr (PH == 1) { mm(I0{}, I0{}, I3{}, I4{}, b0); mm(I0{}, I1{}, I0{}, I4{}, b1); }
            if constexpr (PH == 2) { mm(I1{}, I1{}, I0{}, I4{}, b1); mm(I1{}, I0{}, I0{}, I1{}, b0); }
            if constexpr (PH == 3) mm(I1{}, I0{}, I1{}, I4{}, b0);
        }
        __builtin_amdgcn_s_setprio(0);
    };

    if constexpr (TAB) {
        const unsigned tl = __builtin_amdgcn_readfirstlane(p_lds_addr(smem) + 2 * P_BUF + wave * 2048);
        p_glds2(g_gelu_tab, (unsigned)(wave * 2048 + lane * 16), (unsigned)(wave * 2048 + 1024 + lane * 16), tl, tl + 1024);
    }
    point_at(0);
    issue(I0{}); issue(I1{}); issue(I2{}); issue(I3{});
    issue(I0{}); issue(I1{}); issue(I2{});
    stream_wait(total_kt >= 2);
    __builtin_amdgcn_s_barrier();
    if (wr == 1) __builtin_amdgcn_s_barrier();

#ifdef SSL4GIE_DEBUG_KNOBS
    const bool stamping = ((dbg == 4 && wave == 0) || (dbg == 8 && wave == 4)) && lane == 0 && (blockIdx.x & 15) == 0 && (blockIdx.x >> 4) < NT256_STAMP_WGS;
    auto stamp = [&](int ti, int k) {
        if (stamping && ti < NT256_STAMP_TILES) g_nt256_stamps[blockIdx.x >> 4][ti][k] = __builtin_amdgcn_s_memrealtime();
    };
#else
    auto stamp = [](int, int) {};
#endif
    constexpr bool HAS_BIAS = MODE == SSL4GIE_EPI_BIAS || MODE == SSL4GIE_EPI_BIAS_GELU ||
                              MODE == SSL4GIE_EPI_BIAS_RESIDUAL || MODE == SSL4GIE_EPI_BIAS_GELU_GRAD;
    const unsigned stg_lds = __builtin_amdgcn_readfirstlane(p_lds_addr(smem) + 2 * P_BUF +
                                                            (TAB ? P_TAB_BYTES + wave * 256 : wave * P_STG_WAVE));
    auto issue_bias = [&](int ti) {
        if constexpr (HAS_BIAS) {
            if (e_bias) {
                int col = (tile_of(ti) % tiles_n) * BN + wc * WN + lane;
                col = col < N ? col : N - 1;
                p_glds1_dword(e_bias, (unsigned)col * 4u, stg_lds);
            }
        }
    };
#ifdef SSL4GIE_DEBUG_KNOBS
    if ((dbg == 9 || dbg == 10) && wr == 1) {
        float fake[4] = {0.01f * lane, 0.02f * lane - 0.4f, 0.3f, -0.01f * lane};
        auto chunk = [&]() {
            if (dbg == 10) {
#pragma unroll
                for (int q = 0; q < 4; ++q) {
                    float cdf, xpdf;
                    gelu_parts_fast(fake[q], cdf, xpdf);
                    fake[q] = fake[q] * cdf * 0.5f + (cdf + xpdf) * 0.25f - 0.3f;
                }
            }
        };
        for (int T = 0; T < total_kt; ++T) {
            issue(I3{}); __builtin_amdgcn_s_barrier(); chunk(); __builtin_amdgcn_s_barrier();
            issue(I0{}); __builtin_amdgcn_s_barrier(); chunk(); __builtin_amdgcn_s_barrier();
            issue(I1{}); __builtin_amdgcn_s_barrier(); chunk(); __builtin_amdgcn_s_barrier();
            issue(I2{}); stream_wait(T + 2 < total_kt); __builtin_amdgcn_s_barrier(); chunk();
            __builtin_amdgcn_s_barrier();
        }
        asm volatile("" ::"v"(fake[0] + fake[1] + fake[2] + fake[3]));
        return;
    }
#endif
    int c_kt = 0, c_ti = 0;
    for (int T = 0; T < total_kt; ++T) {
        const int cb = T & 1;
        if (c_kt == 0) {
            stamp(c_ti, 0);
            if (dbg != 7) issue_bias(c_ti);
        }
        if constexpr (PH2) {
#pragma unroll
            for (int ni = 0; ni < 2; ++ni)
#pragma unroll
                for (int ks = 0; ks < 2; ++ks) b0[ni][ks] = ldB(cb, 0, ni, ks);
#pragma unroll
            for (int ni = 0; ni < NI1; ++ni)
#pragma unroll
                for (int ks = 0; ks < 2; ++ks) b1[ni][ks] = ldB(cb, 1, ni, ks);
#pragma unroll
            for (int mi = 0; mi < 4; ++mi)
#pragma unroll
                for (int ks = 0; ks < 2; ++ks) a[mi][ks] = ldA(cb, 0, mi, ks);
            __builtin_amdgcn_sched_barrier(0);
            issue(I3{});
            asm volatile("s_waitcnt lgkmcnt(0)" ::: "memory");
            __builtin_amdgcn_sched_barrier(0);
            __builtin_amdgcn_s_barrier();
            mma(I0{});
            mma(I1{});
            __builtin_amdgcn_sched_barrier(0);
            __builtin_amdgcn_s_barrier();
#pragma unroll
            for (int mi = 0; mi < 4; ++mi)
#pragma unroll
                for (int ks = 0; ks < 2; ++ks) a[mi][ks] = ldA(cb, 1, mi, ks);
            __builtin_amdgcn_sched_barrier(0);
            issue(I0{});
            issue(I1{});
            issue(I2{});
            stream_wait(T + 2 < total_kt);
            asm volatile("s_waitcnt lgkmcnt(0)" ::: "memory");
            __builtin_amdgcn_sched_barrier(0);
            __builtin_amdgcn_s_barrier();
            mma(I2{});
            mma(I3{});
            __builtin_amdgcn_sched_barrier(0);
        } else {
    #pragma unroll
            for (int ni = 0; ni < 2; ++ni)
    #pragma unroll
                for (int ks = 0; ks < 2; ++ks) b0[ni][ks] = ldB(cb, 0, ni, ks);
            __builtin_amdgcn_sched_barrier(0);
    #pragma unroll
            for (int mi = 0; mi < 4; ++mi)
    #pragma unroll
                for (int ks = 0; ks < 2; ++ks) a[mi][ks] = ldA(cb, 0, mi, ks);
            __builtin_amdgcn_sched_barrier(0);
            issue(I3{});
            asm volatile("s_waitcnt lgkmcnt(8)" ::: "memory");
            __builtin_amdgcn_s_barrier();
            mma(I0{});
            __builtin_amdgcn_sched_barrier(0);
            __builtin_amdgcn_s_barrier();
    #pragma unroll
            for (int ni = 0; ni < NI1; ++ni)
    #pragma unroll
                for (int ks = 0; ks < 2; ++ks) b1[ni][ks] = ldB(cb, 1, ni, ks);
            __builtin_amdgcn_sched_barrier(0);
            issue(I0{});
            __builtin_amdgcn_s_barrier();
            mma(I1{});
            __builtin_amdgcn_sched_barrier(0);
            __builtin_amdgcn_s_barrier();
    #pragma unroll
            for (int mi = 0; mi < 4; ++mi)
    #pragma unroll
                for (int ks = 0; ks < 2; ++ks) a[mi][ks] = ldA(cb, 1, mi, ks);
            __builtin_amdgcn_sched_barrier(0);
            issue(I1{});
            __builtin_amdgcn_s_barrier();
            mma(I2{});
            __builtin_amdgcn_sched_barrier(0);
            __builtin_amdgcn_s_barrier();
            issue(I2{});
            stream_wait(T + 2 < total_kt);
            __builtin_amdgcn_s_barrier();
            mma(I3{});
            __builtin_amdgcn_sched_barrier(0);
        }
        if (c_ti > 0 && c_kt == 0) stamp(c_ti - 1, 3);
        if (c_ti > 0 && c_kt == 1) stamp(c_ti - 1, 4);
        if (++c_kt == nk) {
            c_kt = 0;
            const int tile = tile_of(c_ti);
            ++c_ti;
            const int m0 = (tile / tiles_n) * P_BM, n0 = (tile % tiles_n) * BN;
            if (wr == 0) __builtin_amdgcn_s_barrier();
            if constexpr (ROLE != 0 && HAS_BIAS) {
                if (!loader) asm volatile("s_waitcnt vmcnt(0)" ::: "memory");
            }
            stamp(c_ti - 1, 1);
            char* stg = smem + 2 * P_BUF + (TAB ? P_TAB_BYTES + wave * 256 : wave * P_STG_WAVE);
            const bool full = m0 + P_BM <= M && n0 + BN <= N;
#ifdef SSL4GIE_DEBUG_KNOBS
            const float* x_res = e_residual;
            const bf16_t* x_aux = e_aux;
            bf16_t* x_out2 = e_out2;
            TC* x_C = C;
            long long x_ldr = e_ldr;
            int x_rbase = m0 + wr * 128, x_M = M, reps = 1;
            bool x_full = full, skip = false;
            if (dbg == 1 || dbg == 9 || dbg == 10 || ((dbg == 5 || dbg == 6) && wr == 1)) skip = true;
            if (dbg == 2) { x_full = false; x_M = 0; }
            if (dbg == 3) {
                const size_t row = (size_t)(pos % (M > 0 ? M : 1));
                if (x_res) x_res += row * e_ldr;
                if (x_aux) x_aux += row * ldc;
                if (x_out2) x_out2 += row * ldc;
                x_C += row * ldc;
                x_ldr = 0; x_rbase = 0; x_full = true;
            }
            if (dbg == 6 && full) reps = 2;
            if (skip) {
                asm volatile("" ::"v"(acc[0][0][0]), "v"(acc[7][NJ - 1][3]));
            } else if (x_full) {
                for (int rep = 0; rep < reps; ++rep)
                    p_epilogue<TC, MODE, true, STATS, true, NJ>(acc, stg, e_alpha, e_bias, x_res, x_ldr, x_aux, x_out2,
                                                      e_accumulate, x_C, dbg == 3 ? 0 : ldc, x_rbase + rep * 128,
                                                      n0 + wc * WN, x_M, N, lane, e_colstats,
                                                      (stamping && c_ti - 1 < NT256_STAMP_TILES)
                                                          ? &g_nt256_stamps[blockIdx.x >> 4][c_ti - 1][5] : nullptr,
                                                      dbg_prio & 59, !(dbg_prio & 4));
            } else {
                p_epilogue<TC, MODE, false, STATS, true, NJ>(acc, stg, e_alpha, e_bias, x_res, x_ldr, x_aux, x_out2,
                                                   e_accumulate, x_C, ldc, x_rbase, n0 + wc * WN, x_M, N, lane,
                                                   e_colstats, nullptr, dbg_prio & 59, !(dbg_prio & 4));
            }
#else
            if (full)
                p_epilogue<TC, MODE, true, STATS, true, NJ, NTS, TAB>(acc, stg, e_alpha, e_bias, e_residual, e_ldr, e_aux,
                                                  e_out2, e_accumulate, C, ldc, m0 + wr * 128,
                                                  n0 + wc * WN, M, N, lane, e_colstats, nullptr, P_EPI_PRIO_MODE,
                                                  P_EPI_XPOSE_SWAP, smem + 2 * P_BUF);
            else
                p_epilogue<TC, MODE, false, STATS, true, NJ, NTS, TAB>(acc, stg, e_alpha, e_bias, e_residual, e_ldr, e_aux,
                                                   e_out2, e_accumulate, C, ldc, m0 + wr * 128,
                                                   n0 + wc * WN, M, N, lane, e_colstats, nullptr, P_EPI_PRIO_MODE,
                                                   P_EPI_XPOSE_SWAP, smem + 2 * P_BUF);
#endif
            stamp(c_ti - 1, 2);
#pragma unroll
            for (int i = 0; i < 8; ++i)
#pragma unroll
                for (int j = 0; j < NJ; ++j) acc[i][j] = f32x4{0, 0, 0, 0};
            if (wr == 1) __builtin_amdgcn_s_barrier();
        } else {
            __builtin_amdgcn_s_barrier();
        }
    }
    if (wr == 0) __builtin_amdgcn_s_barrier();
}

static int nt256_mode() {
    static int v = -2;
    if (v == -2) {
        const char* s = getenv("SSL4GIE_NT256");
        v = !s ? -1 : (s[0] == '0' ? 0 : 1);
    }
    return v;
}

bool ssl4gie_internal_nt256_ok(const ssl4gie_gemm_desc* d) {
    const int mode = nt256_mode();
    if (mode == 0 && !d->conv) return false;
    if ((!d->conv && (long long)d->M * d->sAm * 2 >= (1LL << 32)) ||
        (long long)d->N * d->sBn * 2 >= (1LL << 32))
        return false;
    if (d->K % P_BK != 0 || d->N % 8 != 0 || d->ldc % 8 != 0) return false;
    const int ep = d->epilogue;
    if (d->colstats && !(d->dtype_c == SSL4GIE_BF16 && ep == SSL4GIE_EPI_NONE && !d->accumulate &&
                         d->N % 8 == 0))
        return false;
    if (!d->C && !d->colstats) return false;
    if (ep == SSL4GIE_EPI_AFFINE_AUX_RELU)
        return !d->conv && d->dtype_c == SSL4GIE_BF16 && d->scale && d->bias && !d->accumulate && d->C;
    if (d->conv)
        return ssl4gie_internal_conv_geom_ok(d->conv) && d->conv->C % P_BK == 0 &&
               d->K == 9 * d->conv->C && (long long)d->M == conv_rows(d->conv) &&
               d->dtype_c == SSL4GIE_BF16 && !d->accumulate &&
               (ep == SSL4GIE_EPI_BIAS || ep == SSL4GIE_EPI_NONE ||
                (ep == SSL4GIE_EPI_RELU_MASK_AUX && d->aux && !d->conv->relu));
    if (d->dtype_c == SSL4GIE_BF16) {
        if (ep == SSL4GIE_EPI_BIAS_RESIDUAL || d->accumulate) return false;
    } else {
        if (ep == SSL4GIE_EPI_BIAS_GELU || ep == SSL4GIE_EPI_DGELU ||
            ep == SSL4GIE_EPI_BIAS_GELU_GRAD || ep == SSL4GIE_EPI_MUL_AUX || ep == SSL4GIE_EPI_RELU_MASK_AUX ||
            ep == SSL4GIE_EPI_ADD_AUX)
            return false;
    }
    if (ep == SSL4GIE_EPI_ADD_AUX) return d->aux != nullptr;
    if (mode == 1 || d->colstats) return true;
    const long long tiles = (long long)((d->M + P_BM - 1) / P_BM) * ((d->N + P_BN - 1) / P_BN);
    return tiles >= 128;
}

static bool nt256_nj2_mode(const ssl4gie_gemm_desc* d) {
#ifdef SSL4GIE_DEBUG_KNOBS
    return false;
#else
    static int on = -1;
    if (on < 0) { const char* s = getenv("SSL4GIE_NT256_NJ2"); on = (s && s[0] == '0') ? 0 : 1; }
    if (!on || d->conv || d->dtype_c != SSL4GIE_BF16) return false;
    const int ep = d->epilogue;
    return ep == SSL4GIE_EPI_NONE || ep == SSL4GIE_EPI_BIAS || ep == SSL4GIE_EPI_ADD_AUX || ep == SSL4GIE_EPI_AFFINE_AUX_RELU;
#endif
}
static int nt256_pick_nj(const ssl4gie_gemm_desc* d, int cus) {
    if (d->conv) return 4;
#ifdef SSL4GIE_DEBUG_KNOBS
    static int forced = -1;
    if (forced < 0) { const char* s = getenv("SSL4GIE_NT256_NJ"); forced = s ? atoi(s) : 0; }
    if (forced == 3 || forced == 4) return forced;
    static int stats4 = -1;
    if (stats4 < 0) { const char* s = getenv("SSL4GIE_NT256_STATS_NJ4"); stats4 = s ? atoi(s) : 0; }
    if (stats4 && d->colstats) return 4;
#endif
    const long long tm = (d->M + P_BM - 1) / P_BM;
    const long long r256 = (tm * ((d->N + 255) / 256) + cus - 1) / cus;
    const long long r192 = (tm * ((d->N + 191) / 192) + cus - 1) / cus;
    int nj = (double)r192 * 0.78 < (double)r256 ? 3 : 4;
    if (d->N <= 128 && nt256_nj2_mode(d)) nj = 2;
    return nj;
}

int ssl4gie_internal_nt256_launch(const ssl4gie_gemm_desc* d, hipStream_t st) {
    const int cus = ssl4gie_internal_compute_cus();
    const int nj = nt256_pick_nj(d, cus);
    const int tm = (d->M + P_BM - 1) / P_BM, tn = (d->N + 64 * nj - 1) / (64 * nj);
    const int ntiles = tm * tn;
    static int balance = -1;
    if (balance < 0) { const char* e = getenv("SSL4GIE_NT_BALANCE"); balance = e ? atoi(e) : 1; }
    int wgs = ntiles < cus ? ntiles : cus;
    if (balance && ntiles > cus) {
        const int rounds = (ntiles + cus - 1) / cus;
        wgs = (ntiles + rounds - 1) / rounds;
    }
    dim3 grid(wgs), block(512);
    static long long stream_m = -2;
    if (stream_m == -2) { const char* s = getenv("SSL4GIE_NT_STREAM_M"); stream_m = s ? atoll(s) : 16384; }
    EpiArgs e{d->alpha, d->epilogue, d->bias, d->residual, d->ldr, d->aux, d->out2, d->accumulate,
              d->colstats, (stream_m >= 0 && d->M >= stream_m) ? 1 : 0};
    if (d->epilogue == SSL4GIE_EPI_AFFINE_AUX_RELU) {
        e.residual = d->scale;
        e.accumulate = d->relu;
    }
    int skip_epi = 0;
    [[maybe_unused]] int role = NT256_DEFAULT_ROLE;
    [[maybe_unused]] bool ph2 = NT256_DEFAULT_PH2;
#ifdef SSL4GIE_DEBUG_KNOBS
    {
        static int k_epi = -1, k_role = -1, k_ph2 = 0;
        if (k_epi < 0) {
            const char* s = getenv("SSL4GIE_NT256_NOEPI");
            k_epi = s ? (atoi(s) & 15) : 0;
            s = getenv("SSL4GIE_NT256_ROLE");
            k_role = s ? (s[0] - '0') : NT256_DEFAULT_ROLE;
            if (k_epi || s) fprintf(stderr, "ssl4gie: DEBUG KNOBS active: NT256_NOEPI=%d NT256_ROLE=%d\n", k_epi, k_role);
            s = getenv("SSL4GIE_NT256_PH2");
            k_ph2 = s ? atoi(s) : (NT256_DEFAULT_PH2 ? 1 : 0);
            s = getenv("SSL4GIE_NT256_PRIO");
            k_epi |= (s ? atoi(s) : P_EPI_PRIO_MODE) << 4;
        }
        skip_epi = k_epi;
        role = k_role;
        ph2 = k_ph2 != 0;
    }
#endif
    static int gelu_tab = -1;
    if (gelu_tab < 0) { const char* s = getenv("SSL4GIE_GELU_TABLE"); gelu_tab = (s && s[0] == '0') ? 0 : 1; }
    ConvK ck{};
    if (d->conv) {
        const int rc = ssl4gie_internal_conv_k(d->conv, &ck);
        if (rc) return rc;
    }
    ProfScope prof(PROF_GEMM_NT, 2.0 * d->M * d->N * d->K, st);
#ifdef SSL4GIE_DEBUG_KNOBS
#define P_LAUNCH(TC_, MODE_)                                                   \
    do {                                                                        \
        if (nj == 3 && ph2) P_LAUNCH_R(TC_, MODE_, 0, false, 0, 3, true);       \
        else if (nj == 3) P_LAUNCH_R(TC_, MODE_, 0, false, 0, 3, false);        \
        else if (role == 1) P_LAUNCH_R(TC_, MODE_, 0, false, 1, 4, false);      \
        else if (ph2) P_LAUNCH_R(TC_, MODE_, 0, false, 0, 4, true);             \
        else P_LAUNCH_R(TC_, MODE_, 0, false, 0, 4, false);                     \
    } while (0)
#else
#define P_LAUNCH(TC_, MODE_)                                                              \
    do {                                                                                   \
        if (nj == 3) P_LAUNCH_R(TC_, MODE_, 0, false, 0, 3, NT256_DEFAULT_PH2);            \
        else P_LAUNCH_R(TC_, MODE_, 0, false, NT256_DEFAULT_ROLE, 4, NT256_DEFAULT_PH2);   \
    } while (0)
#endif
#ifdef SSL4GIE_DEBUG_KNOBS
#define P_LAUNCH2(TC_, MODE_) P_LAUNCH(TC_, MODE_)
#else
#define P_LAUNCH2(TC_, MODE_)  \
    do {                                                                                   \
        if (nj == 2) P_LAUNCH_R(TC_, MODE_, 0, false, 0, 2, NT256_DEFAULT_PH2);            \
        else P_LAUNCH(TC_, MODE_);                                                         \
    } while (0)
#endif
#ifdef SSL4GIE_DEBUG_KNOBS
#define P_LAUNCH_G(MODE_) P_LAUNCH(bf16_t, MODE_)
#else
#define P_LAUNCH_G(MODE_)                                                                                \
    do {                                                                                                  \
        if (nj == 4 && gelu_tab && e.nt_store) P_LAUNCH_KT(bf16_t, MODE_, 0, false, 0, 4, NT256_DEFAULT_PH2, true, true);  \
        else if (nj == 4 && gelu_tab) P_LAUNCH_KT(bf16_t, MODE_, 0, false, 0, 4, NT256_DEFAULT_PH2, false, true);          \
        else P_LAUNCH(bf16_t, MODE_);                                                                     \
    } while (0)
#endif
#define P_LAUNCH_C(TC_, MODE_, CONV_) P_LAUNCH_S(TC_, MODE_, CONV_, false)
#ifdef SSL4GIE_DEBUG_KNOBS
#define P_LAUNCH_S(TC_, MODE_, CONV_, STATS_)                            \
    do {                                                                  \
        if (ph2) P_LAUNCH_R(TC_, MODE_, CONV_, STATS_, 0, 4, true);       \
        else P_LAUNCH_R(TC_, MODE_, CONV_, STATS_, 0, 4, false);          \
    } while (0)
#else
#define P_LAUNCH_S(TC_, MODE_, CONV_, STATS_) P_LAUNCH_R(TC_, MODE_, CONV_, STATS_, 0, 4, NT256_DEFAULT_PH2)
#endif
#ifdef SSL4GIE_DEBUG_KNOBS
#define P_LAUNCH_R(TC_, MODE_, CONV_, STATS_, ROLE_, NJ_, PH2_) P_LAUNCH_K(TC_, MODE_, CONV_, STATS_, ROLE_, NJ_, PH2_, false)
#else
#define P_LAUNCH_R(TC_, MODE_, CONV_, STATS_, ROLE_, NJ_, PH2_)                                        \
    do {                                                                                           \
        if (CONV_ == 0 && !(STATS_) && e.nt_store) P_LAUNCH_K(TC_, MODE_, 0, false, ROLE_, NJ_, PH2_, true); \
        else P_LAUNCH_K(TC_, MODE_, CONV_, STATS_, ROLE_, NJ_, PH2_, false);                       \
    } while (0)
#endif
#define P_LAUNCH_K(TC_, MODE_, CONV_, STATS_, ROLE_, NJ_, PH2_, NTS_) P_LAUNCH_KT(TC_, MODE_, CONV_, STATS_, ROLE_, NJ_, PH2_, NTS_, false)
#define P_LAUNCH_KT(TC_, MODE_, CONV_, STATS_, ROLE_, NJ_, PH2_, NTS_, TAB_)                           \
    do {                                                                                           \
        auto kfn = gemm_bf16_nt256_kernel<TC_, MODE_, CONV_, STATS_, ROLE_, NJ_, PH2_, NTS_, TAB_>; \
        static bool attr_set = false;         \
        if (!attr_set) {                                                                           \
            HIP_RET(hipFuncSetAttribute((const void*)kfn,                                          \
                                        hipFuncAttributeMaxDynamicSharedMemorySize, P_LDS_BYTES)); \
            attr_set = true;                                                                       \
        }                                                                                          \
        hipLaunchKernelGGL(kfn, grid, block, P_LDS_BYTES, st, (const bf16_t*)d->A, d->sAm,         \
                           (const bf16_t*)d->B, d->sBn, (TC_*)d->C, d->ldc, d->M, d->N, d->K, tn,  \
                           ntiles, e, skip_epi, ck);                                                \
    } while (0)
    if (d->colstats) {
        const int cv = d->conv ? (d->conv->relu ? 2 : 1) : 0;
        if (cv == 0 && nj == 3) P_LAUNCH_R(bf16_t, SSL4GIE_EPI_NONE, 0, true, 0, 3, NT256_DEFAULT_PH2);
#ifndef SSL4GIE_DEBUG_KNOBS
        else if (cv == 0 && nj == 2) P_LAUNCH_R(bf16_t, SSL4GIE_EPI_NONE, 0, true, 0, 2, NT256_DEFAULT_PH2);
#endif
        else if (cv == 0) P_LAUNCH_S(bf16_t, SSL4GIE_EPI_NONE, 0, true);
        else if (cv == 1) P_LAUNCH_S(bf16_t, SSL4GIE_EPI_NONE, 1, true);
        else P_LAUNCH_S(bf16_t, SSL4GIE_EPI_NONE, 2, true);
    } else if (d->conv) {
        const bool relu = d->conv->relu != 0, bias = d->epilogue == SSL4GIE_EPI_BIAS;
        if (d->epilogue == SSL4GIE_EPI_RELU_MASK_AUX) P_LAUNCH_C(bf16_t, SSL4GIE_EPI_RELU_MASK_AUX, 1);
        else if (bias && relu) P_LAUNCH_C(bf16_t, SSL4GIE_EPI_BIAS, 2);
        else if (bias) P_LAUNCH_C(bf16_t, SSL4GIE_EPI_BIAS, 1);
        else if (relu) P_LAUNCH_C(bf16_t, SSL4GIE_EPI_NONE, 2);
        else P_LAUNCH_C(bf16_t, SSL4GIE_EPI_NONE, 1);
    } else if (d->dtype_c == SSL4GIE_BF16) {
        switch (d->epilogue) {
            case SSL4GIE_EPI_BIAS: P_LAUNCH2(bf16_t, SSL4GIE_EPI_BIAS); break;
            case SSL4GIE_EPI_BIAS_GELU: P_LAUNCH_G(SSL4GIE_EPI_BIAS_GELU); break;
            case SSL4GIE_EPI_DGELU: P_LAUNCH(bf16_t, SSL4GIE_EPI_DGELU); break;
            case SSL4GIE_EPI_BIAS_GELU_GRAD: P_LAUNCH_G(SSL4GIE_EPI_BIAS_GELU_GRAD); break;
            case SSL4GIE_EPI_MUL_AUX: P_LAUNCH(bf16_t, SSL4GIE_EPI_MUL_AUX); break;
            case SSL4GIE_EPI_ADD_AUX: P_LAUNCH2(bf16_t, SSL4GIE_EPI_ADD_AUX); break;
            case SSL4GIE_EPI_AFFINE_AUX_RELU: P_LAUNCH2(bf16_t, SSL4GIE_EPI_AFFINE_AUX_RELU); break;
            case SSL4GIE_EPI_NONE: P_LAUNCH2(bf16_t, SSL4GIE_EPI_NONE); break;
            default: return ARG_ERR;
        }
    } else {
        switch (d->epilogue) {
            case SSL4GIE_EPI_BIAS: P_LAUNCH(float, SSL4GIE_EPI_BIAS); break;
            case SSL4GIE_EPI_BIAS_RESIDUAL: P_LAUNCH(float, SSL4GIE_EPI_BIAS_RESIDUAL); break;
            case SSL4GIE_EPI_NONE: P_LAUNCH(float, SSL4GIE_EPI_NONE); break;
            default: return ARG_ERR;
        }
    }
#undef P_LAUNCH
#undef P_LAUNCH2
#undef P_LAUNCH_C
#undef P_LAUNCH_S
#undef P_LAUNCH_R
#undef P_LAUNCH_G
#undef P_LAUNCH_KT
    LAUNCH_CHECK();
    return 0;
}
```

Before: 11910 images/sec.

## Add 224- and 160-row GEMM tile variants chosen by wave-quantization cost model

Templates the NT256 GEMM kernel and its epilogues on the number of 16-row MFMA sub-tiles per wave, which allows 224- or 160-row block tiles alongside the 256-row default. A host-side picker estimates per-CU wave-count cost for each tile height, using fixed relative cost factors, and picks a shorter tile when it reduces tail quantization without adding total work. The A-operand loads and the MFMA phase schedule skip the unused rows. The gain is better CU load balance on GEMM shapes that fit poorly, at the cost of lower per-tile arithmetic intensity, more kernel instantiations, and cost constants that may not suit every shape.

```diff
diff --git a/include/ssl4gie_hip.h b/include/ssl4gie_hip.h
--- a/include/ssl4gie_hip.h
+++ b/include/ssl4gie_hip.h
@@ -332,6 +332,7 @@
                       long long n, float smooth, void* workspace, void* stream);
 
 int ssl4gie_debug_nt256_stamps(void* dst, size_t bytes);
+int ssl4gie_debug_nt256_rows(int mi);
 
 typedef struct ssl4gie_ar_handle ssl4gie_ar_handle;
 size_t ssl4gie_allreduce_direct_blob_bytes(void);
diff --git a/ssl4gie_amd/_lib.py b/ssl4gie_amd/_lib.py
--- a/ssl4gie_amd/_lib.py
+++ b/ssl4gie_amd/_lib.py
@@ -180,6 +180,7 @@
     "ssl4gie_conv3x3_weight_pack": (i32, [vp, vp, i32, i32, i32, i32, i32, vp]),
     "ssl4gie_conv3x3_wgrad_unpack": (i32, [vp, vp, i32, i32, i32, i32, vp]),
     "ssl4gie_debug_nt256_stamps": (i32, [vp, sz]),
+    "ssl4gie_debug_nt256_rows": (i32, [i32]),
     "ssl4gie_prof_begin": (i32, [i32]),
     "ssl4gie_prof_collect": (i32, [vp, vp, vp]),
     "ssl4gie_prof_end": (i32, []),
diff --git a/ssl4gie_amd/csrc/gemm256.h b/ssl4gie_amd/csrc/gemm256.h
--- a/ssl4gie_amd/csrc/gemm256.h
+++ b/ssl4gie_amd/csrc/gemm256.h
@@ -101,8 +101,8 @@
     est<NT>((u32x2*)p, r);
 }
 
-template <bool FULL, bool RESID, int NJ = 4, bool NT = false>
-DEVI void p_store_f32(f32x4 (&acc)[8][4], char* stg, const float alpha, const f32x4 bias_t ,
+template <bool FULL, bool RESID, int NJ = 4, bool NT = false, int MI = 8>
+DEVI void p_store_f32(f32x4 (&acc)[MI][4], char* stg, const float alpha, const f32x4 bias_t ,
                       const float* __restrict__ residual, const long long ldr, const bool accumulate,
                       float* __restrict__ C, const long long ldc, int rbase, int cbase, int M, int N,
                       int lane) {
@@ -134,7 +134,7 @@
     };
     put(0);
 #pragma unroll
-    for (int mt = 0; mt < 8; ++mt) {
+    for (int mt = 0; mt < MI; ++mt) {
         f32x4 w[4];
 #pragma unroll
         for (int q = 0; q < 4; ++q) {
@@ -142,7 +142,7 @@
             w[q] = *(const f32x4*)(stg + R * 256 + ((Cc ^ R) << 4));
         }
         __builtin_amdgcn_sched_barrier(0);
-        if (mt + 1 < 8) put(mt + 1);
+        if (mt + 1 < MI) put(mt + 1);
         __builtin_amdgcn_sched_barrier(0);
 #pragma unroll
         for (int q = 0; q < 4; ++q) {
@@ -157,13 +157,13 @@
             }
         }
         if constexpr (RESID) {
-            if (mt + PF < 8) fetch(mt + PF, rs[mt % PF]);
-        }
-    }
-}
-
-template <bool FULL, int AUXF, int NJ = 4, bool NT = false>
-DEVI void p_store_bf16_aux(f32x4 (&acc)[8][4], char* stg, const float alpha,
+            if (mt + PF < MI) fetch(mt + PF, rs[mt % PF]);
+        }
+    }
+}
+
+template <bool FULL, int AUXF, int NJ = 4, bool NT = false, int MI = 8>
+DEVI void p_store_bf16_aux(f32x4 (&acc)[MI][4], char* stg, const float alpha,
                            const bf16_t* __restrict__ aux, bf16_t* __restrict__ C,
                            const long long ldc, int rbase, int cbase, int M, int N, int lane,
                            const float* __restrict__ scale = nullptr, const float* __restrict__ shift = nullptr,
@@ -199,7 +199,7 @@
     };
     put(0);
 #pragma unroll
-    for (int mt = 0; mt < 8; ++mt) {
+    for (int mt = 0; mt < MI; ++mt) {
         f32x4 w[4];
 #pragma unroll
         for (int q = 0; q < 4; ++q) {
@@ -207,7 +207,7 @@
             w[q] = *(const f32x4*)(stg + R * 256 + ((Cc ^ R) << 4));
         }
         __builtin_amdgcn_sched_barrier(0);
-        if (mt + 1 < 8) put(mt + 1);
+        if (mt + 1 < MI) put(mt + 1);
         __builtin_amdgcn_sched_barrier(0);
 #pragma unroll
         for (int q = 0; q < 4; ++q) {
@@ -236,7 +236,7 @@
             }
             if (mine && (FULL || (gm < M && gn < N))) est4<NT>(C + (size_t)gm * ldc + gn, w[q]);
         }
-        if (mt + PF < 8) fetch(mt + PF, ax[mt % PF]);
+        if (mt + PF < MI) fetch(mt + PF, ax[mt % PF]);
     }
 }
 
@@ -280,8 +280,9 @@
     }
 }
 
-template <typename TC, int MODE, bool FULL, bool STATS, bool BIAS_LDS = false, int NJ = 4, bool NT = false, bool TAB = false>
-DEVI void p_epilogue(f32x4 (&acc)[8][4], char* stg, const float alpha,
+template <typename TC, int MODE, bool FULL, bool STATS, bool BIAS_LDS = false, int NJ = 4, bool NT = false, bool TAB = false,
+          int MI = 8>
+DEVI void p_epilogue(f32x4 (&acc)[MI][4], char* stg, const float alpha,
                      const float* __restrict__ bias, const float* __restrict__ residual,
                      const long long ldr, const bf16_t* __restrict__ aux, bf16_t* __restrict__ out2,
                      const int accumulate, TC* __restrict__ C, long long ldc, int rbase, int cbase,
@@ -290,6 +291,7 @@
                      const int prio_mode = P_EPI_PRIO_MODE ,
                      const bool xpose_swap = P_EPI_XPOSE_SWAP ,
                      const char* tab = nullptr ) {
+    static_assert(!STATS || MI == 8, "the column statistics fold whole 128-row blocks");
     const int r16 = lane & 15, g4 = lane >> 4;
     constexpr bool HAS_BIAS = MODE == SSL4GIE_EPI_BIAS || MODE == SSL4GIE_EPI_BIAS_GELU ||
                               MODE == SSL4GIE_EPI_BIAS_RESIDUAL || MODE == SSL4GIE_EPI_BIAS_GELU_GRAD;
@@ -319,13 +321,13 @@
     }
     if constexpr (BIAS_LDS) __builtin_amdgcn_sched_barrier(0);
     if constexpr (sizeof(TC) == 2 && MODE == SSL4GIE_EPI_AFFINE_AUX_RELU) {
-        p_store_bf16_aux<FULL, 5, NJ, NT>(acc, stg, alpha, aux, (bf16_t*)C, ldc, rbase, cbase, M, N, lane,
+        p_store_bf16_aux<FULL, 5, NJ, NT, MI>(acc, stg, alpha, aux, (bf16_t*)C, ldc, rbase, cbase, M, N, lane,
                                       residual , bias , accumulate );
     } else if constexpr (sizeof(TC) == 2 && (MODE == SSL4GIE_EPI_DGELU || MODE == SSL4GIE_EPI_MUL_AUX ||
                                       MODE == SSL4GIE_EPI_RELU_MASK_AUX || MODE == SSL4GIE_EPI_ADD_AUX)) {
         constexpr int AUXF = MODE == SSL4GIE_EPI_DGELU ? 2
                            : (MODE == SSL4GIE_EPI_RELU_MASK_AUX ? 3 : (MODE == SSL4GIE_EPI_ADD_AUX ? 4 : 1));
-        p_store_bf16_aux<FULL, AUXF, NJ, NT>(acc, stg, alpha, aux, (bf16_t*)C, ldc, rbase, cbase, M, N, lane);
+        p_store_bf16_aux<FULL, AUXF, NJ, NT, MI>(acc, stg, alpha, aux, (bf16_t*)C, ldc, rbase, cbase, M, N, lane);
     } else if constexpr (sizeof(TC) == 2) {
         const int R0 = lane >> 3, Cc = lane & 7;
         auto put = [&](int base, int nt, const f32x4& x) {
@@ -399,9 +401,9 @@
             };
             rd(0, qa[0], qb[0]);
 #pragma unroll
-            for (int i = 0; i < 16; ++i) {
+            for (int i = 0; i < 2 * MI; ++i) {
                 const int mt = i >> 1, np = i & 1;
-                if (i + 1 < 16) rd(i + 1, qa[(i + 1) & 1], qb[(i + 1) & 1]);
+                if (i + 1 < 2 * MI) rd(i + 1, qa[(i + 1) & 1], qb[(i + 1) & 1]);
                 unsigned dA[2], gA[2], dB[2], gB[2];
                 p_gelu_tab_finish(qa[i & 1], dA, gA);
                 p_gelu_tab_finish(qb[i & 1], dB, gB);
@@ -436,7 +438,7 @@
         if constexpr (PAIR && NJ == 4 && !TAB) {
             if (xpose_swap) {
 #pragma unroll
-                for (int mt = 0; mt < 8; ++mt) {
+                for (int mt = 0; mt < MI; ++mt) {
                     const int gm = rbase + 16 * mt + r16;
 #pragma unroll
                     for (int np = 0; np < 2; ++np) {
@@ -482,13 +484,13 @@
         prio(0);
         stage(0);
 #pragma unroll
-        for (int mt = 0; mt < 8; ++mt) {
+        for (int mt = 0; mt < MI; ++mt) {
             u32x4 w0[2], w1[2];
             fetch(0, w0);
             if constexpr (PAIR) fetch(2048, w1);
             __builtin_amdgcn_sched_barrier(0);
             prio(mt + 1);
-            if (mt + 1 < 8) stage(mt + 1);
+            if (mt + 1 < MI) stage(mt + 1);
             __builtin_amdgcn_sched_barrier(0);
             store(w0, (bf16_t*)C, mt, true);
             if constexpr (PAIR) store(w1, out2, mt, false);
@@ -514,7 +516,7 @@
             }
         }
     } else {
-        p_store_f32<FULL, MODE == SSL4GIE_EPI_BIAS_RESIDUAL, NJ, NT>(
+        p_store_f32<FULL, MODE == SSL4GIE_EPI_BIAS_RESIDUAL, NJ, NT, MI>(
             acc, stg, alpha, bias_t, residual, ldr, MODE == SSL4GIE_EPI_NONE && accumulate, (float*)C,
             ldc, rbase, cbase, M, N, lane);
     }
diff --git a/ssl4gie_amd/csrc/gemm_nt256.hip b/ssl4gie_amd/csrc/gemm_nt256.hip
--- a/ssl4gie_amd/csrc/gemm_nt256.hip
+++ b/ssl4gie_amd/csrc/gemm_nt256.hip
@@ -24,7 +24,7 @@
 #endif
 
 template <typename TC, int MODE, int CONV, bool STATS = false, int ROLE = 0, int NJ = 4, bool PH2 = false,
-          bool NTS = false , bool TAB = false>
+          bool NTS = false , bool TAB = false, int MI = 8>
 __global__ __launch_bounds__(512, 2) void gemm_bf16_nt256_kernel(
     const bf16_t* __restrict__ A, long long lda, const bf16_t* __restrict__ B, long long ldb,
     TC* __restrict__ C, long long ldc, int M, int N, int K, int tiles_n, int ntiles, EpiArgs e,
@@ -65,8 +65,13 @@
     static_assert(!TAB || (NJ == 4 && ROLE == 0 && CONV == 0 && !STATS && sizeof(TC) == 2 &&
                            (MODE == SSL4GIE_EPI_BIAS_GELU || MODE == SSL4GIE_EPI_BIAS_GELU_GRAD)),
                   "the table form exists for the GELU pair on the 256 x 256 tile");
+    static_assert(MI == 8 || ((MI == 7 || MI == 5) && NJ == 4 && ROLE == 0 && CONV == 0 && !STATS && PH2),
+                  "224 / 160-row tiles: plain operands, ROLE 0, no statistics, two-phase K-tile");
     constexpr int WN = 16 * NJ;
     constexpr int BN = 4 * WN;
+    constexpr int WM = 16 * MI;
+    constexpr int BM = 2 * WM;
+    constexpr int R1 = MI - 4;
 #pragma unroll
     for (int J = 0; J < 4; ++J) vo[J][0] = vo[J][1] = 0;
     yo[0][0] = yo[0][1] = yo[1][0] = yo[1][1] = 0;
@@ -83,7 +88,7 @@
     const int c_cpt = c_C / P_BK;
     auto point_at = [&](int ti) {
         const int tile = tile_of(ti);
-        const int sm0 = (tile / tiles_n) * P_BM, sn0 = (tile % tiles_n) * BN;
+        const int sm0 = (tile / tiles_n) * BM, sn0 = (tile % tiles_n) * BN;
         auto offs = [&](int i, int h, bool is_a) -> unsigned {
             if (NJ == 3 && !is_a && h == 1) {
                 const int lr1 = wave * 8 + (lane >> 3);
@@ -93,7 +98,7 @@
             }
             const int lr = (pbase + i) * 8 + (lane >> 3);
             if (is_a) {
-                int ra = sm0 + (lr >> 6) * 128 + h * 64 + (lr & 63);
+                int ra = sm0 + (lr >> 6) * WM + h * 64 + (lr & 63);
                 ra = ra < M ? ra : M - 1;
                 if constexpr (CONV != 0) return (unsigned)ra;
                 return (unsigned)((long long)ra * lda * 2) + (ROLE == 0 ? co[i] : 0u);
@@ -152,6 +157,8 @@
                 if constexpr (NJ == 2 && J == 2) {
                 } else if constexpr (NJ == 3 && J == 2) {
                     p_glds1(base, vo[J][0], dst - pbase * 1024 + wave * 1024);
+                } else if constexpr (MI < 8 && J == 3) {
+                    if (wc < R1) p_glds2(base, vo[J][0], vo[J][1], dst, dst + 1024);
                 } else if constexpr (ROLE == 0) {
                     p_glds2(base, vo[J][0], vo[J][1], dst, dst + 1024);
                 } else {
@@ -202,9 +209,9 @@
                                 (ks ? ch1 : ch0));
     };
 
-    f32x4 acc[8][4];
-#pragma unroll
-    for (int i = 0; i < 8; ++i)
+    f32x4 acc[MI][4];
+#pragma unroll
+    for (int i = 0; i < MI; ++i)
 #pragma unroll
         for (int j = 0; j < NJ; ++j) acc[i][j] = f32x4{0, 0, 0, 0};
     bf16x8 a[4][2], b0[2][2], b1[2][2];
@@ -236,6 +243,12 @@
         if constexpr (NJ == 2) {
             if constexpr (PH == 0) mm(I0{}, I0{}, I0{}, I4{}, b0);
             if constexpr (PH == 3) mm(I1{}, I0{}, I0{}, I4{}, b0);
+        } else if constexpr (NJ == 4 && MI < 8) {
+            using IR = std::integral_constant<int, R1>;
+            if constexpr (PH == 0) mm(I0{}, I0{}, I0{}, I4{}, b0);
+            if constexpr (PH == 1) mm(I0{}, I1{}, I0{}, IR{}, b1);
+            if constexpr (PH == 2) { mm(I0{}, I1{}, IR{}, I4{}, b1); mm(I1{}, I1{}, I0{}, IR{}, b1); }
+            if constexpr (PH == 3) mm(I1{}, I0{}, I0{}, IR{}, b0);
         } else if constexpr (NJ == 4) {
             if constexpr (PH == 0) mm(I0{}, I0{}, I0{}, I4{}, b0);
             if constexpr (PH == 1) mm(I0{}, I1{}, I0{}, I4{}, b1);
@@ -336,7 +349,7 @@
             __builtin_amdgcn_sched_barrier(0);
             __builtin_amdgcn_s_barrier();
 #pragma unroll
-            for (int mi = 0; mi < 4; ++mi)
+            for (int mi = 0; mi < R1; ++mi)
 #pragma unroll
                 for (int ks = 0; ks < 2; ++ks) a[mi][ks] = ldA(cb, 1, mi, ks);
             __builtin_amdgcn_sched_barrier(0);
@@ -399,21 +412,21 @@
             c_kt = 0;
             const int tile = tile_of(c_ti);
             ++c_ti;
-            const int m0 = (tile / tiles_n) * P_BM, n0 = (tile % tiles_n) * BN;
+            const int m0 = (tile / tiles_n) * BM, n0 = (tile % tiles_n) * BN;
             if (wr == 0) __builtin_amdgcn_s_barrier();
             if constexpr (ROLE != 0 && HAS_BIAS) {
                 if (!loader) asm volatile("s_waitcnt vmcnt(0)" ::: "memory");
             }
             stamp(c_ti - 1, 1);
             char* stg = smem + 2 * P_BUF + (TAB ? P_TAB_BYTES + wave * 256 : wave * P_STG_WAVE);
-            const bool full = m0 + P_BM <= M && n0 + BN <= N;
+            const bool full = m0 + BM <= M && n0 + BN <= N;
 #ifdef SSL4GIE_DEBUG_KNOBS
             const float* x_res = e_residual;
             const bf16_t* x_aux = e_aux;
             bf16_t* x_out2 = e_out2;
             TC* x_C = C;
             long long x_ldr = e_ldr;
-            int x_rbase = m0 + wr * 128, x_M = M, reps = 1;
+            int x_rbase = m0 + wr * WM, x_M = M, reps = 1;
             bool x_full = full, skip = false;
             if (dbg == 1 || dbg == 9 || dbg == 10 || ((dbg == 5 || dbg == 6) && wr == 1)) skip = true;
             if (dbg == 2) { x_full = false; x_M = 0; }
@@ -427,11 +440,11 @@
             }
             if (dbg == 6 && full) reps = 2;
             if (skip) {
-                asm volatile("" ::"v"(acc[0][0][0]), "v"(acc[7][NJ - 1][3]));
+                asm volatile("" ::"v"(acc[0][0][0]), "v"(acc[MI - 1][NJ - 1][3]));
             } else if (x_full) {
                 for (int rep = 0; rep < reps; ++rep)
                     p_epilogue<TC, MODE, true, STATS, true, NJ>(acc, stg, e_alpha, e_bias, x_res, x_ldr, x_aux, x_out2,
-                                                      e_accumulate, x_C, dbg == 3 ? 0 : ldc, x_rbase + rep * 128,
+                                                      e_accumulate, x_C, dbg == 3 ? 0 : ldc, x_rbase + rep * WM,
                                                       n0 + wc * WN, x_M, N, lane, e_colstats,
                                                       (stamping && c_ti - 1 < NT256_STAMP_TILES)
                                                           ? &g_nt256_stamps[blockIdx.x >> 4][c_ti - 1][5] : nullptr,
@@ -444,18 +457,18 @@
 #else
             if (full)
                 p_epilogue<TC, MODE, true, STATS, true, NJ, NTS, TAB>(acc, stg, e_alpha, e_bias, e_residual, e_ldr, e_aux,
-                                                  e_out2, e_accumulate, C, ldc, m0 + wr * 128,
+                                                  e_out2, e_accumulate, C, ldc, m0 + wr * WM,
                                                   n0 + wc * WN, M, N, lane, e_colstats, nullptr, P_EPI_PRIO_MODE,
                                                   P_EPI_XPOSE_SWAP, smem + 2 * P_BUF);
             else
                 p_epilogue<TC, MODE, false, STATS, true, NJ, NTS, TAB>(acc, stg, e_alpha, e_bias, e_residual, e_ldr, e_aux,
-                                                   e_out2, e_accumulate, C, ldc, m0 + wr * 128,
+                                                   e_out2, e_accumulate, C, ldc, m0 + wr * WM,
                                                    n0 + wc * WN, M, N, lane, e_colstats, nullptr, P_EPI_PRIO_MODE,
                                                    P_EPI_XPOSE_SWAP, smem + 2 * P_BUF);
 #endif
             stamp(c_ti - 1, 2);
 #pragma unroll
-            for (int i = 0; i < 8; ++i)
+            for (int i = 0; i < MI; ++i)
 #pragma unroll
                 for (int j = 0; j < NJ; ++j) acc[i][j] = f32x4{0, 0, 0, 0};
             if (wr == 1) __builtin_amdgcn_s_barrier();
@@ -538,10 +551,65 @@
     return nj;
 }
 
+static const double kNtRowCost[9] = {0, 0, 0, 0, 0, 0.74, 0, 0.95, 1.0};
+static int g_nt256_rows = -1;
+extern "C" int ssl4gie_debug_nt256_rows(int mi) {
+    REQUIRE(mi == 0 || mi == 8 || mi == 7 || mi == 5);
+    g_nt256_rows = mi;
+    return 0;
+}
+static int nt256_rows_knob() {
+    if (g_nt256_rows < 0) {
+        const char* s = getenv("SSL4GIE_NT256_ROWS");
+        int v = 0;
+        if (s && s[0] == '0') v = 8;
+#ifdef SSL4GIE_DEBUG_KNOBS
+        if (s && (atoi(s) == 7 || atoi(s) == 5)) v = atoi(s);
+#endif
+        g_nt256_rows = v;
+    }
+    return g_nt256_rows;
+}
+static int nt256_pick_mi(const ssl4gie_gemm_desc* d, int cus, int nj, bool served) {
+    const int knob = nt256_rows_knob();
+    if (!served || knob == 8) return 8;
+    if (knob == 7 || knob == 5) return knob;
+    if (nj == 2) return 8;
+    const long long tn4 = (d->N + 255) / 256;
+    const long long t8 = (d->M + P_BM - 1) / P_BM * ((d->N + 64 * nj - 1) / (64 * nj));
+    const double c8 = nj == 3 ? 0.78 : 1.0;
+    double best = (double)((t8 + cus - 1) / cus) * c8;
+    const double work = (double)t8 * c8;
+    int mi = 8;
+    for (int m : {7, 5}) {
+        const long long t = (d->M + 32 * m - 1) / (32 * m) * tn4;
+        const double c = (double)((t + cus - 1) / cus) * kNtRowCost[m];
+        if (c < best && (double)t * kNtRowCost[m] <= work) { best = c; mi = m; }
+    }
+    return mi;
+}
+
 int ssl4gie_internal_nt256_launch(const ssl4gie_gemm_desc* d, hipStream_t st) {
     const int cus = ssl4gie_internal_compute_cus();
-    const int nj = nt256_pick_nj(d, cus);
-    const int tm = (d->M + P_BM - 1) / P_BM, tn = (d->N + 64 * nj - 1) / (64 * nj);
+    [[maybe_unused]] int role = NT256_DEFAULT_ROLE;
+    [[maybe_unused]] bool ph2 = NT256_DEFAULT_PH2;
+#ifdef SSL4GIE_DEBUG_KNOBS
+    {
+        const char* s = getenv("SSL4GIE_NT256_ROLE");
+        role = s ? (s[0] - '0') : NT256_DEFAULT_ROLE;
+        s = getenv("SSL4GIE_NT256_PH2");
+        ph2 = s ? atoi(s) != 0 : NT256_DEFAULT_PH2;
+    }
+#endif
+    static int gelu_tab = -1;
+    if (gelu_tab < 0) { const char* s = getenv("SSL4GIE_GELU_TABLE"); gelu_tab = (s && s[0] == '0') ? 0 : 1; }
+    const bool gelu_pair = d->epilogue == SSL4GIE_EPI_BIAS_GELU || d->epilogue == SSL4GIE_EPI_BIAS_GELU_GRAD;
+    int nj = nt256_pick_nj(d, cus);
+    const bool rows_served = !d->conv && !d->colstats && role == 0 && ph2 &&
+                             d->epilogue != SSL4GIE_EPI_AFFINE_AUX_RELU && (!gelu_pair || (gelu_tab && nj == 4));
+    const int mi = nt256_pick_mi(d, cus, nj, rows_served);
+    if (mi < 8) nj = 4;
+    const int tm = (d->M + 32 * mi - 1) / (32 * mi), tn = (d->N + 64 * nj - 1) / (64 * nj);
     const int ntiles = tm * tn;
     static int balance = -1;
     if (balance < 0) { const char* e = getenv("SSL4GIE_NT_BALANCE"); balance = e ? atoi(e) : 1; }
@@ -560,29 +628,20 @@
         e.accumulate = d->relu;
     }
     int skip_epi = 0;
-    [[maybe_unused]] int role = NT256_DEFAULT_ROLE;
-    [[maybe_unused]] bool ph2 = NT256_DEFAULT_PH2;
 #ifdef SSL4GIE_DEBUG_KNOBS
     {
-        static int k_epi = -1, k_role = -1, k_ph2 = 0;
+        static int k_epi = -1;
         if (k_epi < 0) {
             const char* s = getenv("SSL4GIE_NT256_NOEPI");
             k_epi = s ? (atoi(s) & 15) : 0;
-            s = getenv("SSL4GIE_NT256_ROLE");
-            k_role = s ? (s[0] - '0') : NT256_DEFAULT_ROLE;
-            if (k_epi || s) fprintf(stderr, "ssl4gie: DEBUG KNOBS active: NT256_NOEPI=%d NT256_ROLE=%d\n", k_epi, k_role);
-            s = getenv("SSL4GIE_NT256_PH2");
-            k_ph2 = s ? atoi(s) : (NT256_DEFAULT_PH2 ? 1 : 0);
+            if (k_epi || getenv("SSL4GIE_NT256_ROLE"))
+                fprintf(stderr, "ssl4gie: DEBUG KNOBS active: NT256_NOEPI=%d NT256_ROLE=%d\n", k_epi, role);
             s = getenv("SSL4GIE_NT256_PRIO");
             k_epi |= (s ? atoi(s) : P_EPI_PRIO_MODE) << 4;
         }
         skip_epi = k_epi;
-        role = k_role;
-        ph2 = k_ph2 != 0;
-    }
-#endif
-    static int gelu_tab = -1;
-    if (gelu_tab < 0) { const char* s = getenv("SSL4GIE_GELU_TABLE"); gelu_tab = (s && s[0] == '0') ? 0 : 1; }
+    }
+#endif
     ConvK ck{};
     if (d->conv) {
         const int rc = ssl4gie_internal_conv_k(d->conv, &ck);
@@ -592,17 +651,30 @@
 #ifdef SSL4GIE_DEBUG_KNOBS
 #define P_LAUNCH(TC_, MODE_)                                                   \
     do {                                                                        \
-        if (nj == 3 && ph2) P_LAUNCH_R(TC_, MODE_, 0, false, 0, 3, true);       \
+        if (mi == 7) P_LAUNCH_KT(TC_, MODE_, 0, false, 0, 4, true, false, false, 7); \
+        else if (mi == 5) P_LAUNCH_KT(TC_, MODE_, 0, false, 0, 4, true, false, false, 5); \
+        else if (nj == 3 && ph2) P_LAUNCH_R(TC_, MODE_, 0, false, 0, 3, true);  \
         else if (nj == 3) P_LAUNCH_R(TC_, MODE_, 0, false, 0, 3, false);        \
         else if (role == 1) P_LAUNCH_R(TC_, MODE_, 0, false, 1, 4, false);      \
         else if (ph2) P_LAUNCH_R(TC_, MODE_, 0, false, 0, 4, true);             \
         else P_LAUNCH_R(TC_, MODE_, 0, false, 0, 4, false);                     \
     } while (0)
 #else
-#define P_LAUNCH(TC_, MODE_)                                                              \
+#define P_LAUNCH8(TC_, MODE_)                                          \
     do {                                                                                   \
         if (nj == 3) P_LAUNCH_R(TC_, MODE_, 0, false, 0, 3, NT256_DEFAULT_PH2);            \
         else P_LAUNCH_R(TC_, MODE_, 0, false, NT256_DEFAULT_ROLE, 4, NT256_DEFAULT_PH2);   \
+    } while (0)
+#define P_LAUNCH_M(TC_, MODE_, MI_, TAB_)  \
+    do {                                                                                   \
+        if (e.nt_store) P_LAUNCH_KT(TC_, MODE_, 0, false, 0, 4, NT256_DEFAULT_PH2, true, TAB_, MI_);  \
+        else P_LAUNCH_KT(TC_, MODE_, 0, false, 0, 4, NT256_DEFAULT_PH2, false, TAB_, MI_);            \
+    } while (0)
+#define P_LAUNCH(TC_, MODE_)                                                              \
+    do {                                                                                   \
+        if (mi == 7) P_LAUNCH_M(TC_, MODE_, 7, false);                                     \
+        else if (mi == 5) P_LAUNCH_M(TC_, MODE_, 5, false);                                \
+        else P_LAUNCH8(TC_, MODE_);                                                        \
     } while (0)
 #endif
 #ifdef SSL4GIE_DEBUG_KNOBS
@@ -619,9 +691,11 @@
 #else
 #define P_LAUNCH_G(MODE_)                                                                                \
     do {                                                                                                  \
-        if (nj == 4 && gelu_tab && e.nt_store) P_LAUNCH_KT(bf16_t, MODE_, 0, false, 0, 4, NT256_DEFAULT_PH2, true, true);  \
-        else if (nj == 4 && gelu_tab) P_LAUNCH_KT(bf16_t, MODE_, 0, false, 0, 4, NT256_DEFAULT_PH2, false, true);          \
-        else P_LAUNCH(bf16_t, MODE_);                                                                     \
+        if (mi == 7) P_LAUNCH_M(bf16_t, MODE_, 7, true);       \
+        else if (mi == 5) P_LAUNCH_M(bf16_t, MODE_, 5, true);                                                        \
+        else if (nj == 4 && gelu_tab && e.nt_store) P_LAUNCH_KT(bf16_t, MODE_, 0, false, 0, 4, NT256_DEFAULT_PH2, true, true, 8); \
+        else if (nj == 4 && gelu_tab) P_LAUNCH_KT(bf16_t, MODE_, 0, false, 0, 4, NT256_DEFAULT_PH2, false, true, 8);          \
+        else P_LAUNCH8(bf16_t, MODE_);                                                                    \
     } while (0)
 #endif
 #define P_LAUNCH_C(TC_, MODE_, CONV_) P_LAUNCH_S(TC_, MODE_, CONV_, false)
@@ -643,10 +717,10 @@
         else P_LAUNCH_K(TC_, MODE_, CONV_, STATS_, ROLE_, NJ_, PH2_, false);                       \
     } while (0)
 #endif
-#define P_LAUNCH_K(TC_, MODE_, CONV_, STATS_, ROLE_, NJ_, PH2_, NTS_) P_LAUNCH_KT(TC_, MODE_, CONV_, STATS_, ROLE_, NJ_, PH2_, NTS_, false)
-#define P_LAUNCH_KT(TC_, MODE_, CONV_, STATS_, ROLE_, NJ_, PH2_, NTS_, TAB_)                           \
+#define P_LAUNCH_K(TC_, MODE_, CONV_, STATS_, ROLE_, NJ_, PH2_, NTS_) P_LAUNCH_KT(TC_, MODE_, CONV_, STATS_, ROLE_, NJ_, PH2_, NTS_, false, 8)
+#define P_LAUNCH_KT(TC_, MODE_, CONV_, STATS_, ROLE_, NJ_, PH2_, NTS_, TAB_, MI_)                      \
     do {                                                                                           \
-        auto kfn = gemm_bf16_nt256_kernel<TC_, MODE_, CONV_, STATS_, ROLE_, NJ_, PH2_, NTS_, TAB_>; \
+        auto kfn = gemm_bf16_nt256_kernel<TC_, MODE_, CONV_, STATS_, ROLE_, NJ_, PH2_, NTS_, TAB_, MI_>; \
         static bool attr_set = false;         \
         if (!attr_set) {                                                                           \
             HIP_RET(hipFuncSetAttribute((const void*)kfn,                                          \
@@ -694,6 +768,8 @@
         }
     }
 #undef P_LAUNCH
+#undef P_LAUNCH8
+#undef P_LAUNCH_M
 #undef P_LAUNCH2
 #undef P_LAUNCH_C
 #undef P_LAUNCH_S
```

New measurement: 11900 images/sec (median of 3 runs). About the same (-0.1%).
